# nikola3794/normal-clustering-nerf

Measured on AMD Instinct MI355X. Metric: training rays/sec (+ samples/sec), higher is better.
Workload: dtype fp32 (march/composite/losses); fp16-operand MFMA with fp32 accumulate in the field MLP; 1 GPU; configs[1]+[2]: full training step, 8192 rays/GPU, normal clustering on; rays_per_gpu=8192, global_batch=8192, grid=128, max_samples=1024, parallelism=dp1, grid_update_every_16=True

## Files before the change

normal-clustering-nerf_amd/csrc/optim.hip:

```cpp
#include <algorithm>
#include "workgroup.h"
#include "../../include/ncnerf.h"

namespace ncn {

constexpr int SUMSQ_BLOCKS = 1024;

__global__ __launch_bounds__(256) void sumsq_kernel(const float* __restrict__ x, int64_t n, float* __restrict__ part,
                                                    int* __restrict__ step_inc) {
    __shared__ float red[4];
    if (step_inc && blockIdx.x == 0 && threadIdx.x == 0) *step_inc += 1;
    float s = 0.f;
    const int64_t n4 = n / 4;
    const float4* x4 = (const float4*)x;
    for (int64_t i = (int64_t)blockIdx.x * 256 + threadIdx.x; i < n4; i += (int64_t)gridDim.x * 256) {
        const float4 v = x4[i];
        s = fmaf(v.x, v.x, s); s = fmaf(v.y, v.y, s); s = fmaf(v.z, v.z, s); s = fmaf(v.w, v.w, s);
    }
    if (blockIdx.x == 0)
        for (int64_t i = n4 * 4 + threadIdx.x; i < n; i += 256) s = fmaf(x[i], x[i], s);
    s = block_sum<256>(s, red);
    if (threadIdx.x == 0) part[blockIdx.x] = s;
}

__device__ __forceinline__ float clip_coef(const float* __restrict__ part, float max_norm) {
    __shared__ float c_s;
    if (threadIdx.x < 64) {
        float s = 0.f;
        for (int i = threadIdx.x; i < SUMSQ_BLOCKS; i += 64) s += part[i];
        s = wave_sum(s);
        if (threadIdx.x == 0) {
            const float norm = sqrtf(s);
            const float c = max_norm / (norm + 1e-6f);
            c_s = max_norm > 0.f ? fminf(c, 1.0f) : 1.0f;
        }
    }
    __syncthreads();
    return c_s;
}

__global__ __launch_bounds__(256) void adam_kernel(float* __restrict__ p, const float* __restrict__ g,
                                                   float* __restrict__ m, float* __restrict__ v, int64_t n,
                                                   const float* __restrict__ part, float max_norm, float lr, float b1,
                                                   float b2, float eps, float wd, float bc1, float bc2,
                                                   const float* __restrict__ lr_dev, const int* __restrict__ step_dev) {
    const float cf = part ? clip_coef(part, max_norm) : 1.0f;
    if (lr_dev) lr = *lr_dev;
    if (step_dev) {
        const float st = (float)*step_dev;
        bc1 = 1.0f - powf(b1, st);
        bc2 = 1.0f - powf(b2, st);
    }
    auto upd = [&](float& pi, float gr, float& mi, float& vi) {
        const float gi = gr * cf;
        mi = b1 * mi + (1.f - b1) * gi;
        vi = b2 * vi + (1.f - b2) * gi * gi;
        const float denom = sqrtf(vi / bc2) + eps;
        pi = pi - lr * ((mi / bc1) / denom + wd * pi);
    };
    const int64_t tid = (int64_t)blockIdx.x * 256 + threadIdx.x, nth = (int64_t)gridDim.x * 256;
    const bool vec = (((uintptr_t)p | (uintptr_t)g | (uintptr_t)m | (uintptr_t)v) & 15) == 0;
    const int64_t n4 = vec ? n / 4 : 0;
    for (int64_t i = tid; i < n4; i += nth) {
        float4 P = ((float4*)p)[i], M = ((float4*)m)[i], V = ((float4*)v)[i];
        const float4 G = ((const float4*)g)[i];
        upd(P.x, G.x, M.x, V.x);
        upd(P.y, G.y, M.y, V.y);
        upd(P.z, G.z, M.z, V.z);
        upd(P.w, G.w, M.w, V.w);
        ((float4*)p)[i] = P;
        ((float4*)m)[i] = M;
        ((float4*)v)[i] = V;
    }
    for (int64_t i = 4 * n4 + tid; i < n; i += nth) upd(p[i], g[i], m[i], v[i]);
}

#ifndef NCN_ADAM_BLOCKS
#define NCN_ADAM_BLOCKS 256
#endif
#ifndef NCN_ADAM_UNROLL
#define NCN_ADAM_UNROLL 12
#endif
constexpr int ADAM_BLOCKS = NCN_ADAM_BLOCKS;
constexpr int ADAM_THREADS = 1024;
constexpr int ADAM_UNROLL = NCN_ADAM_UNROLL;
__global__ __launch_bounds__(ADAM_THREADS) void adam_prep_kernel(const float* __restrict__ g, int64_t n, float gscale,
                                                               float max_norm, double b1, double b2, float lr,
                                                               const float* __restrict__ lr_dev,
                                                               int* __restrict__ step_dev, float* __restrict__ work,
                                                               float* __restrict__ amp, const int* __restrict__ gate) {
    float* part = work;
    unsigned* cnt = (unsigned*)(work + ADAM_BLOCKS);
    float* sc = work + ADAM_BLOCKS + 4;
    __shared__ float red[ADAM_THREADS / 64];
    const int64_t n4 = n / 4, stride = (int64_t)gridDim.x * ADAM_THREADS;
    const float4* g4 = (const float4*)g;
    float s = 0.f;
    for (int64_t b = (int64_t)blockIdx.x * ADAM_THREADS + threadIdx.x; b < n4; b += ADAM_UNROLL * stride) {
        float4 x[ADAM_UNROLL];
#pragma unroll
        for (int u = 0; u < ADAM_UNROLL; u++) x[u] = b + u * stride < n4 ? g4[b + u * stride] : make_float4(0, 0, 0, 0);
#pragma unroll
        for (int u = 0; u < ADAM_UNROLL; u++) {
            s = fmaf(x[u].x, x[u].x, s); s = fmaf(x[u].y, x[u].y, s); s = fmaf(x[u].z, x[u].z, s); s = fmaf(x[u].w, x[u].w, s);
        }
    }
    if (blockIdx.x == 0)
        for (int64_t i = 4 * n4 + threadIdx.x; i < n; i += ADAM_THREADS) s = fmaf(g[i], g[i], s);
    if (!last_block_arrive(&part[blockIdx.x], block_sum<ADAM_THREADS>(s, red), cnt)) return;
    if (threadIdx.x < 64) {
        float q[ADAM_BLOCKS / 64];
#pragma unroll
        for (int u = 0; u < ADAM_BLOCKS / 64; u++) {
            const int i = u * 64 + threadIdx.x;
            q[u] = i < (int)gridDim.x ? __hip_atomic_load(&part[i], __ATOMIC_RELAXED, __HIP_MEMORY_SCOPE_AGENT) : 0.f;
        }
        float t = 0.f;
#pragma unroll
        for (int u = 0; u < ADAM_BLOCKS / 64; u++) t += q[u];
        t = wave_sum(t);
        if (threadIdx.x == 0) {
            const float c = max_norm / (sqrtf(t) * gscale + 1e-6f);
            const bool gated_off = gate && *gate == 0;
            const bool skip = gated_off || (amp && !isfinite(t));
            if (amp && !gated_off) {
                float tr = skip ? 0.f : amp[1] + 1.f;
                float scale = skip ? amp[0] * 0.5f : amp[0];
                if (tr >= (float)NCN_AMP_GROWTH_INTERVAL) {
                    scale *= 2.f;
                    tr = 0.f;
                }
                amp[0] = scale;
                amp[1] = tr;
            }
            const int st = *step_dev + (skip ? 0 : 1);
            *step_dev = st;
            sc[4] = skip ? 1.f : 0.f;
            sc[0] = (max_norm > 0.f ? fminf(c, 1.0f) : 1.0f) * gscale;
            sc[1] = (float)(1.0 - pow(b1, (double)st));
            sc[2] = (float)(1.0 - pow(b2, (double)st));
            sc[3] = lr_dev ? *lr_dev : lr;
            *cnt = 0u;
        }
    }
}
template <int PK>
__device__ __forceinline__ void adam_pack1(int64_t e, float x, const int32_t* __restrict__ pinv, int64_t poff,
                                           int64_t n, void* __restrict__ packed) {
    if (PK == 0 || e < poff || e >= n) return;
    const int64_t w = e - poff;
    const int2 q = ((const int2*)pinv)[w];
    if (PK == 1) {
        const _Float16 h = (_Float16)x;
        if (q.x >= 0) ((_Float16*)packed)[q.x] = h;
        if (q.y >= 0) ((_Float16*)packed)[q.y] = h;
    } else {
        const __bf16 h = (__bf16)x;
        if (q.x >= 0) ((__bf16*)packed)[q.x] = h;
        if (q.y >= 0) ((__bf16*)packed)[q.y] = h;
    }
}
template <bool ZERO, int PK>
__global__ __launch_bounds__(256) void adam_apply_kernel(float* __restrict__ p, float* __restrict__ g,
                                                         float* __restrict__ m, float* __restrict__ v, int64_t n,
                                                         int64_t n0, float b1, float b2, float eps, float wd0,
                                                         float wd1, const float* __restrict__ sc,
                                                         const int32_t* __restrict__ pinv, int64_t poff,
                                                         void* __restrict__ packed) {
    const float cf = sc[0], bc1 = sc[1], bc2 = sc[2], lr = sc[3];
    if (sc[4] != 0.f) {
        if (PK) {
            const int64_t tid = (int64_t)blockIdx.x * 256 + threadIdx.x, nth = (int64_t)gridDim.x * 256;
            for (int64_t e = poff + tid; e < n; e += nth) adam_pack1<PK>(e, p[e], pinv, poff, n, packed);
        }
        if (ZERO) {
            const int64_t tid = (int64_t)blockIdx.x * 256 + threadIdx.x, nth = (int64_t)gridDim.x * 256;
            for (int64_t i = tid; i < n / 4; i += nth) ((float4*)g)[i] = make_float4(0.f, 0.f, 0.f, 0.f);
            for (int64_t i = 4 * (n / 4) + tid; i < n; i += nth) g[i] = 0.f;
        }
        return;
    }
    auto upd = [&](float& pi, float gr, float& mi, float& vi, float wd) {
        const float gi = gr * cf;
        mi = b1 * mi + (1.f - b1) * gi;
        vi = b2 * vi + (1.f - b2) * gi * gi;
        const float denom = sqrtf(vi / bc2) + eps;
        pi = pi - lr * ((mi / bc1) / denom + wd * pi);
    };
    auto upd_tail = [&](float& pi, float gr, float& mi, float& vi, float wd) {
#pragma clang fp contract(off)
        const float gi = gr * cf;
        mi = fmaf(b1, mi, (1.f - b1) * gi);
        vi = fmaf(b2, vi, ((1.f - b2) * gi) * gi);
        const float denom = sqrtf(vi / bc2) + eps;
        pi = fmaf(-lr, fmaf(wd, pi, (mi / bc1) / denom), pi);
    };
    const int64_t n4 = n / 4, tid = (int64_t)blockIdx.x * 256 + threadIdx.x, nth = (int64_t)gridDim.x * 256;
#pragma unroll 2
    for (int64_t i = tid; i < n4; i += nth) {
        float4 P = ((float4*)p)[i], M = ((float4*)m)[i], V = ((float4*)v)[i];
        const float4 G = ((const float4*)g)[i];
        const int64_t e = 4 * i;
        upd(P.x, G.x, M.x, V.x, e < n0 ? wd0 : wd1);
        upd(P.y, G.y, M.y, V.y, e + 1 < n0 ? wd0 : wd1);
        upd(P.z, G.z, M.z, V.z, e + 2 < n0 ? wd0 : wd1);
        upd(P.w, G.w, M.w, V.w, e + 3 < n0 ? wd0 : wd1);
        ((float4*)p)[i] = P;
        ((float4*)m)[i] = M;
        ((float4*)v)[i] = V;
        if (PK && e + 3 >= poff) {
            adam_pack1<PK>(e, P.x, pinv, poff, n, packed);
            adam_pack1<PK>(e + 1, P.y, pinv, poff, n, packed);
            adam_pack1<PK>(e + 2, P.z, pinv, poff, n, packed);
            adam_pack1<PK>(e + 3, P.w, pinv, poff, n, packed);
        }
        if (ZERO && (G.x != 0.f || G.y != 0.f || G.z != 0.f || G.w != 0.f))
            ((float4*)g)[i] = make_float4(0.f, 0.f, 0.f, 0.f);
    }
    for (int64_t i = 4 * n4 + tid; i < n; i += nth) {
        upd_tail(p[i], g[i], m[i], v[i], i < n0 ? wd0 : wd1);
        adam_pack1<PK>(i, p[i], pinv, poff, n, packed);
        if (ZERO) g[i] = 0.f;
    }
}
constexpr int NCN_STEP_MAX_BUFS = 8;
struct StepCopies {
    const unsigned char* src[NCN_STEP_MAX_BUFS];
    unsigned char* dst[NCN_STEP_MAX_BUFS];
    int64_t bytes[NCN_STEP_MAX_BUFS];
};
__global__ __launch_bounds__(256) void step_inputs_kernel(StepCopies c, int nb, int64_t* step_dst, int64_t step,
                                                         int* flag_dst, int flag) {
    if (step_dst && blockIdx.x == 0 && threadIdx.x == 0) *step_dst = step;
    if (flag_dst && blockIdx.x == 0 && threadIdx.x == 0) *flag_dst = flag;
    const int64_t tid = (int64_t)blockIdx.x * 256 + threadIdx.x, nth = (int64_t)gridDim.x * 256;
    for (int b = 0; b < nb; b++) {
        const bool al = (((uintptr_t)c.src[b] | (uintptr_t)c.dst[b]) & 15) == 0;
        const int64_t n16 = al ? c.bytes[b] / 16 : 0;
        for (int64_t i = tid; i < n16; i += nth) ((uint4*)c.dst[b])[i] = ((const uint4*)c.src[b])[i];
        for (int64_t i = 16 * n16 + tid; i < c.bytes[b]; i += nth) c.dst[b][i] = c.src[b][i];
    }
}

__global__ __launch_bounds__(256) void grad_pack_f16_kernel(const float* __restrict__ g, int64_t n,
                                                            const float* __restrict__ scale, int world,
                                                            _Float16* __restrict__ w) {
    const float s = scale ? *scale : 1.f, wf = (float)world;
    auto wire = [&](float x) { return (_Float16)((float)(_Float16)(x * s) / wf); };
    const int64_t n8 = n / 8, stride = (int64_t)gridDim.x * 256;
    for (int64_t i = (int64_t)blockIdx.x * 256 + threadIdx.x; i < n8; i += stride) {
        const float4 a = ((const float4*)g)[2 * i], b = ((const float4*)g)[2 * i + 1];
        typedef _Float16 h8 __attribute__((ext_vector_type(8)));
        const h8 o = {wire(a.x), wire(a.y), wire(a.z), wire(a.w), wire(b.x), wire(b.y), wire(b.z), wire(b.w)};
        ((h8*)w)[i] = o;
    }
    for (int64_t i = 8 * n8 + (int64_t)blockIdx.x * 256 + threadIdx.x; i < n; i += stride) w[i] = wire(g[i]);
}
__global__ __launch_bounds__(256) void grad_unpack_f16_kernel(const _Float16* __restrict__ w, int64_t n,
                                                              const float* __restrict__ scale, float* __restrict__ g) {
    const float inv = scale ? 1.f / *scale : 1.f;
    const int64_t n8 = n / 8, stride = (int64_t)gridDim.x * 256;
    typedef _Float16 h8 __attribute__((ext_vector_type(8)));
    for (int64_t i = (int64_t)blockIdx.x * 256 + threadIdx.x; i < n8; i += stride) {
        const h8 v = ((const h8*)w)[i];
        ((float4*)g)[2 * i] = make_float4((float)v[0] * inv, (float)v[1] * inv, (float)v[2] * inv, (float)v[3] * inv);
        ((float4*)g)[2 * i + 1] = make_float4((float)v[4] * inv, (float)v[5] * inv, (float)v[6] * inv, (float)v[7] * inv);
    }
    for (int64_t i = 8 * n8 + (int64_t)blockIdx.x * 256 + threadIdx.x; i < n; i += stride) g[i] = (float)w[i] * inv;
}

}

using namespace ncn;

extern "C" {

int ncn_grad_pack_f16(const float* grad, int64_t n, const float* scale, int world, uint16_t* wire, void* stream) {
    if (n <= 0) return 0;
    NCN_REQUIRE(world >= 1, hipErrorInvalidValue, "ncn_grad_pack_f16: world must be >= 1");
    NCN_REQUIRE(((((uintptr_t)grad) & 15) | (((uintptr_t)wire) & 15)) == 0, hipErrorInvalidValue,
                "ncn_grad_pack_f16: grad and wire must be 16-byte aligned");
    const int blocks = (int)std::min<int64_t>(std::max<int64_t>(1, cdiv(n, 2048)), 4096);
    hipLaunchKernelGGL(grad_pack_f16_kernel, dim3(blocks), dim3(256), 0, (hipStream_t)stream, grad, n, scale,
                       world, (_Float16*)wire);
    NCN_LAUNCH_CHECK("ncn_grad_pack_f16");
    return 0;
}

int ncn_grad_unpack_f16(const uint16_t* wire, int64_t n, const float* scale, float* grad, void* stream) {
    if (n <= 0) return 0;
    NCN_REQUIRE(((((uintptr_t)grad) & 15) | (((uintptr_t)wire) & 15)) == 0, hipErrorInvalidValue,
                "ncn_grad_unpack_f16: grad and wire must be 16-byte aligned");
    const int blocks = (int)std::min<int64_t>(std::max<int64_t>(1, cdiv(n, 2048)), 4096);
    hipLaunchKernelGGL(grad_unpack_f16_kernel, dim3(blocks), dim3(256), 0, (hipStream_t)stream, (const _Float16*)wire,
                       n, scale, grad);
    NCN_LAUNCH_CHECK("ncn_grad_unpack_f16");
    return 0;
}

int ncn_step_inputs(int n_bufs, const void* const* src, void* const* dst, const int64_t* n_bytes, int64_t* step_dst,
                    int64_t step, int32_t* flag_dst, int32_t flag, void* stream) {
    NCN_REQUIRE(n_bufs >= 0 && n_bufs <= NCN_STEP_MAX_BUFS, hipErrorInvalidValue,
                "ncn_step_inputs: at most 8 buffers");
    StepCopies c{};
    int64_t total = 0;
    for (int b = 0; b < n_bufs; b++) {
        NCN_REQUIRE(n_bytes[b] >= 0 && (n_bytes[b] == 0 || (src[b] && dst[b])), hipErrorInvalidValue,
                    "ncn_step_inputs: null buffer");
        c.src[b] = (const unsigned char*)src[b];
        c.dst[b] = (unsigned char*)dst[b];
        c.bytes[b] = n_bytes[b];
        total += n_bytes[b];
    }
    const int grid = (int)std::max<int64_t>(1, std::min<int64_t>(256, (total / 16 + 255) / 256));
    hipLaunchKernelGGL(step_inputs_kernel, dim3(grid), dim3(256), 0, (hipStream_t)stream, c, n_bufs, step_dst, step,
                       flag_dst, flag);
    NCN_LAUNCH_CHECK("ncn_step_inputs");
    return 0;
}

int ncn_sumsq(const float* x, int64_t n, float* out_partial, int* step_inc, void* stream) {
    hipLaunchKernelGGL(sumsq_kernel, dim3(SUMSQ_BLOCKS), dim3(256), 0, (hipStream_t)stream, x, n, out_partial,
                       step_inc);
    NCN_LAUNCH_CHECK("ncn_sumsq");
    return 0;
}

int ncn_adam(float* params, const float* grads, float* exp_avg, float* exp_avg_sq, int64_t n,
             const float* sumsq_partial, float max_norm, float lr, float beta1, float beta2, float eps,
             float weight_decay, int step, const float* lr_dev, const int* step_dev, void* stream) {
    if (n <= 0) return 0;
    NCN_REQUIRE(step >= 1 || step_dev, hipErrorInvalidValue, "ncn_adam: step must be >= 1");
    const float bc1 = 1.0f - powf(beta1, (float)std::max(step, 1)), bc2 = 1.0f - powf(beta2, (float)std::max(step, 1));
    const int blocks = (int)std::min<int64_t>(cdiv(n, 1024), 2048);
    hipLaunchKernelGGL(adam_kernel, dim3(blocks), dim3(256), 0, (hipStream_t)stream, params, grads, exp_avg,
                       exp_avg_sq, n, sumsq_partial, max_norm, lr, beta1, beta2, eps, weight_decay, bc1, bc2, lr_dev,
                       step_dev);
    NCN_LAUNCH_CHECK("ncn_adam");
    return 0;
}

}

template <int PK>
static void launch_apply(int zero, int blocks, hipStream_t st, float* params, float* grads, float* exp_avg,
                         float* exp_avg_sq, int64_t n, int64_t n_group0, double beta1, double beta2, float eps,
                         float wd0, float wd1, const float* sc, const int32_t* pinv, int64_t poff, void* packed) {
    if (zero)
        hipLaunchKernelGGL((adam_apply_kernel<true, PK>), dim3(blocks), dim3(256), 0, st, params, grads, exp_avg,
                           exp_avg_sq, n, n_group0, (float)beta1, (float)beta2, eps, wd0, wd1, sc, pinv, poff, packed);
    else
        hipLaunchKernelGGL((adam_apply_kernel<false, PK>), dim3(blocks), dim3(256), 0, st, params, grads, exp_avg,
                           exp_avg_sq, n, n_group0, (float)beta1, (float)beta2, eps, wd0, wd1, sc, pinv, poff, packed);
}

static int adam_step_impl(float* params, float* grads, float* exp_avg, float* exp_avg_sq, int64_t n, int64_t n_group0,
                          float grad_scale, float max_norm, float lr, double beta1, double beta2, float eps, float wd0,
                          float wd1, const float* lr_dev, int* step_dev, float* work, int zero_grads,
                          float* amp_state, const int* gate, const int32_t* pinv, int64_t poff, void* packed, int pk,
                          void* stream) {
    if (n <= 0) return 0;
    NCN_REQUIRE(((((uintptr_t)params) | ((uintptr_t)grads) | ((uintptr_t)exp_avg) | ((uintptr_t)exp_avg_sq)) & 15) == 0,
                hipErrorInvalidValue, "ncn_adam_step: buffers must be 16-byte aligned");
    NCN_REQUIRE(step_dev != nullptr && work != nullptr, hipErrorInvalidValue,
                "ncn_adam_step: needs the device step counter and the work buffer");
    const int prep_blocks = (int)std::min<int64_t>(ADAM_BLOCKS, std::max<int64_t>(1, cdiv(n / 4, ADAM_THREADS * 4)));
    hipLaunchKernelGGL(adam_prep_kernel, dim3(prep_blocks), dim3(ADAM_THREADS), 0, (hipStream_t)stream, grads, n,
                       grad_scale, max_norm, beta1, beta2, lr, lr_dev, step_dev, work, amp_state, gate);
    NCN_LAUNCH_CHECK("ncn_adam_step (prep)");
    const int blocks = (int)std::min<int64_t>(std::max<int64_t>(1, cdiv(n, 2048)), 16384);
    const float* sc = work + ADAM_BLOCKS + 4;
    const hipStream_t st = (hipStream_t)stream;
    if (pk == 0)
        launch_apply<0>(zero_grads, blocks, st, params, grads, exp_avg, exp_avg_sq, n, n_group0, beta1, beta2, eps, wd0,
                        wd1, sc, nullptr, 0, nullptr);
    else if (pk == 1)
        launch_apply<1>(zero_grads, blocks, st, params, grads, exp_avg, exp_avg_sq, n, n_group0, beta1, beta2, eps, wd0,
                        wd1, sc, pinv, poff, packed);
    else
        launch_apply<2>(zero_grads, blocks, st, params, grads, exp_avg, exp_avg_sq, n, n_group0, beta1, beta2, eps, wd0,
                        wd1, sc, pinv, poff, packed);
    NCN_LAUNCH_CHECK("ncn_adam_step");
    return 0;
}

extern "C" {

int ncn_adam_step(float* params, float* grads, float* exp_avg, float* exp_avg_sq, int64_t n, int64_t n_group0,
                  float grad_scale, float max_norm, float lr, double beta1, double beta2, float eps, float wd0, float wd1,
                  const float* lr_dev, int* step_dev, float* work, int zero_grads, float* amp_state, const int* gate,
                  void* stream) {
    return adam_step_impl(params, grads, exp_avg, exp_avg_sq, n, n_group0, grad_scale, max_norm, lr, beta1, beta2, eps,
                          wd0, wd1, lr_dev, step_dev, work, zero_grads, amp_state, gate, nullptr, 0, nullptr, 0, stream);
}

int ncn_adam_step_packed(float* params, float* grads, float* exp_avg, float* exp_avg_sq, int64_t n, int64_t n_group0,
                         float grad_scale, float max_norm, float lr, double beta1, double beta2, float eps, float wd0,
                         float wd1, const float* lr_dev, int* step_dev, float* work, int zero_grads, float* amp_state,
                         const int* gate, const int32_t* pack_inv, int64_t pack_off, uint16_t* packed, int pack_prec,
                         void* stream) {
    NCN_REQUIRE(pack_inv && packed && (pack_prec == NCN_PREC_F16 || pack_prec == NCN_PREC_BF16) && pack_off >= 0 &&
                    n - pack_off == NCN_FIELD_NW && (((uintptr_t)pack_inv) & 7) == 0,
                hipErrorInvalidValue, "ncn_adam_step_packed: pack_inv/packed/pack_prec/pack_off invalid");
    return adam_step_impl(params, grads, exp_avg, exp_avg_sq, n, n_group0, grad_scale, max_norm, lr, beta1, beta2, eps,
                          wd0, wd1, lr_dev, step_dev, work, zero_grads, amp_state, gate, pack_inv, pack_off, packed,
                          pack_prec == NCN_PREC_F16 ? 1 : 2, stream);
}

int64_t ncn_adam_step_work_floats(void) { return ADAM_BLOCKS + 12; }

}
```

normal-clustering-nerf_amd/csrc/vren_march_pack.h:

```cpp
#pragma once
#include "vren_march_wave.h"
#include "workgroup.h"

namespace ncn {

__global__ __launch_bounds__(1024) void march_train_scan_kernel(const int32_t* __restrict__ counts, int64_t R,
                                                                int64_t* __restrict__ rays_a,
                                                                int32_t* __restrict__ counter) {
    __shared__ int wave_tot[16];
    const int tid = threadIdx.x;
    int carry = 0;
    for (int64_t base = 0; base < R; base += 4096) {
        const int64_t i0 = base + (int64_t)tid * 4;
        int c[4];
        int local = 0;
#pragma unroll
        for (int j = 0; j < 4; j++) {
            c[j] = (i0 + j < R) ? counts[i0 + j] : 0;
            local += c[j];
        }
        int run = block_excl_sweep<1024>(local, carry, wave_tot);
#pragma unroll
        for (int j = 0; j < 4; j++) {
            const int64_t i = i0 + j;
            if (i < R) {
                rays_a[3 * i] = i;
                rays_a[3 * i + 1] = run;
                rays_a[3 * i + 2] = c[j];
            }
            run += c[j];
        }
    }
    if (tid == 0) {
        counter[0] = carry;
        counter[1] = (int32_t)R;
    }
}

__device__ __forceinline__ void copy_slab_row(const float* __restrict__ sx, const float* __restrict__ st,
                                              const float* __restrict__ sd, const float (&d3)[3], int k0, int n,
                                              int64_t start, int lane, float* __restrict__ xyzs,
                                              float* __restrict__ dirs, float* __restrict__ deltas,
                                              float* __restrict__ ts) {
    for (int k = 3 * k0 + lane; k < 3 * n; k += 64) {
        xyzs[3 * start + k] = sx[k];
        dirs[3 * start + k] = d3[k % 3];
    }
    for (int k = k0 + lane; k < n; k += 64) {
        ts[start + k] = st[k];
        deltas[start + k] = sd[k];
    }
}

__global__ __launch_bounds__(256) void march_train_pack_kernel(
    const float* __restrict__ rays_d, const int64_t* __restrict__ rays_a, int64_t R, int max_samples,
    const float* __restrict__ slab_xyz, const float* __restrict__ slab_t, const float* __restrict__ slab_dt,
    float* __restrict__ xyzs, float* __restrict__ dirs, float* __restrict__ deltas, float* __restrict__ ts) {
    const int lane = threadIdx.x & 63;
    const int64_t n = __builtin_amdgcn_readfirstlane((int)(blockIdx.x * 4 + (threadIdx.x >> 6)));
    if (n >= R) return;
    const int64_t ray = rays_a[3 * n], start = rays_a[3 * n + 1];
    const int cnt = (int)rays_a[3 * n + 2];
    const float d3[3] = {rays_d[3 * ray], rays_d[3 * ray + 1], rays_d[3 * ray + 2]};
    copy_slab_row(slab_xyz + ray * (int64_t)max_samples * 3, slab_t + ray * (int64_t)max_samples,
                  slab_dt + ray * (int64_t)max_samples, d3, 0, cnt, start, lane, xyzs, dirs, deltas, ts);
}

__global__ __launch_bounds__(256) void march_train_place_kernel(
    const float* __restrict__ rays_d, int64_t R, int max_samples, const int32_t* __restrict__ counts,
    const int32_t* __restrict__ wg_sum, const float* __restrict__ slab_xyz, const float* __restrict__ slab_t,
    const float* __restrict__ slab_dt, int64_t* __restrict__ rays_a, float* __restrict__ xyzs,
    float* __restrict__ dirs, float* __restrict__ deltas, float* __restrict__ ts, int32_t* __restrict__ counter) {
    __shared__ int red[4][3];
    const int lane = threadIdx.x & 63, wv = threadIdx.x >> 6;
    const int b = blockIdx.x;
    int v[PLACE_MAX_WG / 256];
#pragma unroll
    for (int u = 0; u < PLACE_MAX_WG / 256; u++) {
        const int i = u * 256 + threadIdx.x;
        v[u] = i < (int)gridDim.x ? wg_sum[i] : 0;
    }
    const int64_t r0 = __builtin_amdgcn_readfirstlane((int)(b * 4 + wv));
    const bool live = r0 < R;
    const int64_t r = live ? r0 : R - 1;
    const int n = live ? counts[r] : 0;
    const float d3[3] = {rays_d[3 * r], rays_d[3 * r + 1], rays_d[3 * r + 2]};
    const float* sx = slab_xyz + r * (int64_t)max_samples * 3;
    const float* st = slab_t + r * (int64_t)max_samples;
    const float* sd = slab_dt + r * (int64_t)max_samples;
    constexpr int PF = 4;
    float px[3 * PF], pt[PF], pd[PF];
#pragma unroll
    for (int q = 0; q < 3 * PF; q++) px[q] = q * 64 + lane < 3 * n ? sx[q * 64 + lane] : 0.f;
#pragma unroll
    for (int q = 0; q < PF; q++) {
        pt[q] = q * 64 + lane < n ? st[q * 64 + lane] : 0.f;
        pd[q] = q * 64 + lane < n ? sd[q * 64 + lane] : 0.f;
    }
    int pre[3] = {0, 0, 0};
#pragma unroll
    for (int u = 0; u < PLACE_MAX_WG / 256; u++) {
        const int i = u * 256 + threadIdx.x;
        const int nl = (int)((unsigned)v[u] >> 26);
        if (i < b) {
            pre[0] += v[u] & ((1 << 26) - 1);
            pre[1] += nl;
        }
        pre[2] += nl;
    }
    block_sum<3, 256>(pre, red);
    int start = pre[0];
    const int long_before = pre[1], long_total = pre[2];
    __syncthreads();
    int* const len = &red[0][0];
    if (lane == 0) len[wv] = n;
    __syncthreads();
    int lw = 0;
    for (int w = 0; w < wv; w++) {
        start += len[w];
        lw += len[w] > PLACE_LONG;
    }
    const int64_t row = n > PLACE_LONG ? (int64_t)(long_before + lw)
                                       : (int64_t)long_total + (4 * (int64_t)b - long_before) + (wv - lw);
    if (b == (int)gridDim.x - 1 && threadIdx.x == 0) {
        counter[0] = start + len[0] + len[1] + len[2] + len[3];
        counter[1] = (int32_t)R;
    }
    if (!live) return;
    if (lane == 0) {
        rays_a[3 * row] = r;
        rays_a[3 * row + 1] = start;
        rays_a[3 * row + 2] = n;
    }
    float* ox = xyzs + 3 * (int64_t)start;
    float* od = dirs + 3 * (int64_t)start;
#pragma unroll
    for (int q = 0; q < 3 * PF; q++) {
        const int k = q * 64 + lane;
        if (k < 3 * n) {
            ox[k] = px[q];
            od[k] = d3[k % 3];
        }
    }
#pragma unroll
    for (int q = 0; q < PF; q++) {
        const int k = q * 64 + lane;
        if (k < n) {
            ts[start + k] = pt[q];
            deltas[start + k] = pd[q];
        }
    }
    copy_slab_row(sx, st, sd, d3, PF * 64, n, start, lane, xyzs, dirs, deltas, ts);
}

}
```

normal-clustering-nerf_amd/csrc/vren_march_wave.h:

```cpp
#pragma once
#include "vren_aabb.h"
#include "vren_march.h"

namespace ncn {


template <int P>
__device__ __forceinline__ float march_chain(float cb, float dt, int lane, float (&c)[P]) {
    constexpr int L = 64 * P;
#pragma unroll
    for (int j = 0; j < P; j++) c[j] = cb;
    int j0 = 0;
    float v = cb;
    for (;;) {
        const uint32_t bv = __float_as_uint(v);
        const float v1 = v + dt;
        const uint32_t b1 = __float_as_uint(v1);
        uint32_t r1 = b1 - bv, r = 0;
        int K;
        float vn;
        if ((bv >> 23) != (b1 >> 23) || bv == 0u) {
            K = 0;
            vn = v1;
        } else {
            const float v2 = v1 + dt;
            const uint32_t b2 = __float_as_uint(v2);
            if ((b2 >> 23) != (b1 >> 23)) {
                K = 1;
                vn = v2;
            } else {
                r = b2 - b1;
                if (r == 0u) {
#pragma unroll
                    for (int j = 0; j < P; j++)
                        if (lane + 64 * j > j0) c[j] = v;
                    return v;
                }
                const uint32_t room = (bv | 0x7FFFFFu) - bv - r1;
                K = (uint64_t)room >= (uint64_t)(L - 1) * r ? L : (int)(room / r + 1u);
                vn = __uint_as_float(bv + r1 + (uint32_t)(K - 1) * r) + dt;
            }
        }
#pragma unroll
        for (int j = 0; j < P; j++) {
            const int i = lane + 64 * j;
            if (i > j0 && i <= j0 + K) c[j] = __uint_as_float(bv + r1 + (uint32_t)(i - j0 - 1) * r);
        }
        if (j0 + K >= L) return __uint_as_float(bv + r1 + (uint32_t)(L - j0 - 1) * r);
        const int J = j0 + K + 1;
        if (J == L) return vn;
#pragma unroll
        for (int j = 0; j < P; j++)
            if (lane + 64 * j == J) c[j] = vn;
        j0 = J;
        v = vn;
    }
}

__device__ __forceinline__ float lane_f(float v, int idx) { return __int_as_float(__builtin_amdgcn_ds_bpermute(idx << 2, __float_as_int(v))); }
__device__ __forceinline__ int lane_i(int v, int idx) { return __builtin_amdgcn_ds_bpermute(idx << 2, v); }

__device__ __forceinline__ int march_skip_lane(float c, float T, float dt, int lane) {
    const float q = ceilf((T - c) / dt);
    int j = lane + (int)fminf(fmaxf(q, 1.0f), 65.0f);
    if (j > 64) j = 64;
    const float cm = lane_f(c, min(j - 1, 63));
    const float cj = lane_f(c, min(j, 63));
    if (j - 1 > lane && cm >= T) j -= 1;
    else if (j < 64 && cj < T) j += 1;
    const float cm2 = lane_f(c, min(j - 1, 63));
    const float cj2 = lane_f(c, min(j, 63));
    const bool ok = (j - 1 == lane || cm2 < T) && (j == 64 || cj2 >= T);
    if (__ballot(!ok)) {
        int p = lane;
#pragma unroll
        for (int st = 32; st >= 1; st >>= 1) {
            const int qn = p + st;
            const float cq = lane_f(c, min(qn, 63));
            if (qn <= 63 && cq < T) p = qn;
        }
        j = p + 1;
    }
    return j;
}

__device__ __forceinline__ uint64_t march_visited(int nxt, int s, int lane) {
    int J[6];
    J[0] = nxt;
#pragma unroll
    for (int i = 1; i < 6; i++) {
        const int v = lane_i(J[i - 1], min(J[i - 1], 63));
        J[i] = J[i - 1] >= 64 ? 64 : v;
    }
    int cur = s;
#pragma unroll
    for (int i = 5; i >= 0; i--) {
        const int v = lane_i(J[i], min(cur, 63));
        const int cand = cur >= 64 ? 64 : v;
        if (cand <= lane) cur = cand;
    }
    return __ballot(cur == lane && lane >= s);
}

template <bool ONE_CASCADE, int P>
__device__ __forceinline__ int march_walk_wave(const MarchConst& m, const uint8_t* __restrict__ bitfield, float ox,
                                               float oy, float oz, float dx, float dy, float dz, float t1, float t2,
                                               float noise_r, float dt, int lane, float* __restrict__ sx,
                                               float* __restrict__ st, float* __restrict__ sd) {
    const float dxi = 1.0f / dx, dyi = 1.0f / dy, dzi = 1.0f / dz;
    int n = 0;
    if (t1 >= 0) {
        t1 = fmaf(dt, noise_r, t1);
        float cb = t1;
        bool pend = false, done = false;
        float ptgt = 0.f;
        int s = 0;
        for (int it = 0; it < (1 << 16) && !done; it++) {
            float c[P];
            const float cnext = march_chain<P>(cb, dt, lane, c);
            float X[P], Y[P], Z[P], tgt[P];
            bool occ[P];
#pragma unroll
            for (int j = 0; j < P; j++) {
                X[j] = fmaf(c[j], dx, ox);
                Y[j] = fmaf(c[j], dy, oy);
                Z[j] = fmaf(c[j], dz, oz);
                int nx, ny, nz;
                float mip_bound;
                uint32_t cbi = 0xFFFFFFFFu, cbv = 0;
                occ[j] = probe<ONE_CASCADE>(m, bitfield, X[j], Y[j], Z[j], dt, nx, ny, nz, mip_bound, cbi, cbv);
                tgt[j] = skip_target(m, c[j], X[j], Y[j], Z[j], dx, dy, dz, dxi, dyi, dzi, nx, ny, nz, mip_bound);
            }
#pragma unroll
            for (int j = 0; j < P; j++) {
                if (done) break;
                const uint64_t lt_m = __ballot(c[j] < t2);
                const uint64_t occ_m = __ballot(occ[j]);
                if (pend) {
                    const uint64_t mm = __ballot(c[j] >= ptgt);
                    if (!mm) continue;
                    s = __builtin_ctzll(mm);
                    pend = false;
                }
                const int skip = march_skip_lane(c[j], tgt[j], dt, lane);
                const int nxt = !(c[j] < t2) ? 64 : (occ[j] ? lane + 1 : skip);
                const uint64_t vis = march_visited(nxt, s, lane);
                const uint64_t term = vis & ~lt_m;
                uint64_t emit = vis & occ_m & lt_m;
                const int room = m.max_samples - n;
                if (__popcll(emit) >= room) {
                    uint64_t e2 = emit;
                    for (int q = 1; q < room; q++) e2 &= e2 - 1;
                    const int last = __builtin_ctzll(e2);
                    emit &= (last == 63) ? ~0ull : ((2ull << last) - 1);
                    done = true;
                }
                if (term) {
                    emit &= (1ull << __builtin_ctzll(term)) - 1;
                    done = true;
                }
                if (emit) {
                    if ((emit >> lane) & 1) {
                        const int k = n + (int)__builtin_amdgcn_mbcnt_hi((uint32_t)(emit >> 32),
                                                                       __builtin_amdgcn_mbcnt_lo((uint32_t)emit, 0));
                        sx[3 * k] = X[j];
                        sx[3 * k + 1] = Y[j];
                        sx[3 * k + 2] = Z[j];
                        st[k] = c[j];
                        sd[k] = dt;
                    }
                    n += __popcll(emit);
                }
                if (!done) {
                    const int lastv = 63 - __builtin_clzll(vis);
                    if ((occ_m >> lastv) & 1) {
                        s = 0;
                    } else {
                        pend = true;
                        ptgt = __int_as_float(__builtin_amdgcn_readlane(__float_as_int(tgt[j]), lastv));
                    }
                }
            }
            cb = cnext;
        }
    }
    return n;
}

template <bool ONE_CASCADE, int P>
__global__ __launch_bounds__(256) void march_train_wave_kernel(
    const float* __restrict__ rays_o, const float* __restrict__ rays_d, const float* __restrict__ hits_t,
    const float* __restrict__ noise, int64_t R, const uint8_t* __restrict__ bitfield, int cascades, float scale,
    int G, int max_samples, int32_t* __restrict__ counts, float* __restrict__ slab_xyz,
    float* __restrict__ slab_t, float* __restrict__ slab_dt) {
    const int lane = threadIdx.x & 63;
    const int64_t r = __builtin_amdgcn_readfirstlane((int)(blockIdx.x * 4 + (threadIdx.x >> 6)));
    if (r >= R) return;
    const MarchConst m = make_march_const(cascades, scale, 0.0f, G, max_samples, scale);
    const float t1 = hits_t[2 * r];
    const int n = march_walk_wave<ONE_CASCADE, P>(
        m, bitfield, rays_o[3 * r], rays_o[3 * r + 1], rays_o[3 * r + 2], rays_d[3 * r], rays_d[3 * r + 1],
        rays_d[3 * r + 2], t1, hits_t[2 * r + 1], t1 >= 0 ? noise[r] : 0.f, calc_dt(m, 0.0f), lane,
        slab_xyz + r * (int64_t)max_samples * 3, slab_t + r * (int64_t)max_samples, slab_dt + r * (int64_t)max_samples);
    if (lane == 0) counts[r] = n;
}

__device__ __forceinline__ float march_uniform(uint64_t seed, uint64_t ctr, uint32_t r) {
    uint64_t z = seed + 0x9E3779B97F4A7C15ull * (ctr * 0x100000001B3ull + r + 1u);
    z = (z ^ (z >> 30)) * 0xBF58476D1CE4E5B9ull;
    z = (z ^ (z >> 27)) * 0x94D049BB133111EBull;
    z ^= z >> 31;
    return (float)(uint32_t)(z >> 40) * (1.0f / 16777216.0f);
}

constexpr int PLACE_MAX_WG = 256 * 16;
constexpr int PLACE_LONG = 256;

template <bool ONE_CASCADE, int P>
__global__ __launch_bounds__(256) void march_train_walk2_kernel(
    const float* __restrict__ rays_o, const float* __restrict__ rays_d, int64_t R, float cx, float cy, float cz,
    float hx, float hy, float hz, float near_distance, const float* __restrict__ noise, uint64_t seed,
    const int64_t* __restrict__ rng_ctr, const uint8_t* __restrict__ bitfield, int cascades, float scale, int G,
    int max_samples, float* __restrict__ slab_xyz, float* __restrict__ slab_t, float* __restrict__ slab_dt,
    int32_t* __restrict__ counts, int32_t* __restrict__ wg_sum) {
    __shared__ int cnt_s[4];
    const int lane = threadIdx.x & 63, wv = threadIdx.x >> 6;
    const int64_t r0 = __builtin_amdgcn_readfirstlane((int)(blockIdx.x * 4 + wv));
    const bool live = r0 < R;
    const int64_t r = live ? r0 : R - 1;
    const MarchConst m = make_march_const(cascades, scale, 0.0f, G, max_samples, scale);
    const float o[3] = {rays_o[3 * r], rays_o[3 * r + 1], rays_o[3 * r + 2]};
    const float d[3] = {rays_d[3 * r], rays_d[3 * r + 1], rays_d[3 * r + 2]};
    const float c3[3] = {cx, cy, cz}, h3[3] = {hx, hy, hz};
    const float inv[3] = {1.0f / d[0], 1.0f / d[1], 1.0f / d[2]};
    float t1, t2;
    slab_test(o, inv, c3, h3, t1, t2);
    if (t2 > 0) t1 = fmaxf(t1, 0.0f);
    else { t1 = -1.0f; t2 = -1.0f; }
    if (t1 >= 0.0f && t1 < near_distance) t1 = near_distance;
    float nz = 0.f;
    if (t1 >= 0) nz = noise ? noise[r] : march_uniform(seed, rng_ctr ? (uint64_t)*rng_ctr : 0ull, (uint32_t)r);
    int n = 0;
    if (live)
        n = march_walk_wave<ONE_CASCADE, P>(m, bitfield, o[0], o[1], o[2], d[0], d[1], d[2], t1, t2, nz,
                                            calc_dt(m, 0.0f), lane, slab_xyz + r * (int64_t)max_samples * 3,
                                            slab_t + r * (int64_t)max_samples, slab_dt + r * (int64_t)max_samples);
    if (lane == 0) {
        cnt_s[wv] = n;
        if (live) counts[r] = n;
    }
    __syncthreads();
    if (threadIdx.x == 0) {
        int nl = 0;
#pragma unroll
        for (int w = 0; w < 4; w++) nl += cnt_s[w] > PLACE_LONG;
        wg_sum[blockIdx.x] = (cnt_s[0] + cnt_s[1] + cnt_s[2] + cnt_s[3]) | (nl << 26);
    }
}

}
```

normal-clustering-nerf_amd/ncnerf_amd/_lib.py:

```python
import ctypes
import operator
import os
import re

import torch

_HERE = os.path.dirname(os.path.abspath(__file__))
LIB_PATH = os.environ.get("NCN_LIB_PATH") or os.path.join(_HERE, "libncnerf.so")
INCLUDE_DIR = os.path.join(os.path.dirname(os.path.dirname(_HERE)), "include")
_DERIVED = {
    "ncnerf.h": "the binding",
    "ncnerf_metrics.h": "the binding of the validation metrics",
    "ncnerf_geom.h": "the binding of the geometry supervision",
    "ncnerf_mesh.h": "the binding of the isosurface extraction",
    "ncnerf_heads.h": "the binding of the semantic / normal heads",
    "ncnerf_sem.h": "the binding of the semantic metrics",
    "ncnerf_input_grad.h": "the binding of the split backward's direction gradient",
}
HEADERS = tuple(_DERIVED)

P = ctypes.c_void_p
I64 = ctypes.c_int64
I32 = ctypes.c_int
U32 = ctypes.c_uint32
F32 = ctypes.c_float
F64 = ctypes.c_double
U64 = ctypes.c_uint64


class NcnError(RuntimeError):
    pass


_RESTYPES = {"int": ctypes.c_int, "int64_t": I64, "const char*": ctypes.c_char_p}
_SCALARS = {"int": I32, "int32_t": I32, "int64_t": I64, "uint32_t": U32, "uint64_t": U64, "float": F32, "double": F64}
_POINTEES = {"void": 0, "float": 4, "double": 8, "int": 4, "int32_t": 4, "int64_t": 8, "uint8_t": 1, "uint16_t": 2,
             "uint32_t": 4}
_DECL = re.compile(r"(const\s+char\s*\*|int64_t|int)\s*(\w+)\s*\(([^()]*)\)")
_PARAM = re.compile(r"(?:const\s+)?(\w+)(?:\s*((?:\*\s*(?:const\b\s*)?)+)|\s+)(\w+)")


def parse_header(text):
    text = re.sub(r"/\*.*?\*/|//[^\n]*", " ", text, flags=re.S)
    if re.search(r"^\s*#.*\\$", text, flags=re.M):
        raise ValueError("ncnerf.h grammar: a preprocessor line is continued with a backslash")
    text = re.sub(r"^\s*#.*$", "", text, flags=re.M)
    text, n_extern = re.subn(r'extern\s+"C"\s*\{', "", text)
    text = text.strip()
    if n_extern == 1 and text.endswith("}"):
        text = text[:-1]
    *decls, rest = text.split(";")
    if rest.strip():
        raise ValueError(f"ncnerf.h grammar: no ';' after {' '.join(rest.split())!r}")
    out = {}
    for decl in decls:
        decl = " ".join(decl.split())
        m = _DECL.fullmatch(decl)
        if m is None:
            raise ValueError(f"ncnerf.h grammar: not `int|int64_t|const char* name(params)`: {decl!r}")
        ret, name, params = m.groups()
        if name in out:
            raise ValueError(f"ncnerf.h grammar: {name} is declared twice")
        plist = []
        for p in ([] if params.strip() in ("", "void") else params.split(",")):
            pm = _PARAM.fullmatch(p.strip())
            if pm is None or pm.group(3) in _POINTEES or pm.group(3) in _SCALARS or pm.group(3) == "const":
                raise ValueError(f"ncnerf.h grammar: parameter {p.strip()!r} of {decl!r} is not `type name`")
            base, stars, pname = pm.group(1), (pm.group(2) or "").count("*"), pm.group(3)
            if stars == 0 and base in _SCALARS:
                plist.append((base, 0, pname))
            elif stars == 1 and base in _POINTEES:
                plist.append(("ptr", _POINTEES[base], pname))
            elif stars == 2 and base == "void":
                plist.append(("ptr", 8, pname))
            else:
                raise ValueError(f"ncnerf.h grammar: unknown type in parameter {p.strip()!r} of {decl!r}")
        out[name] = ("const char*" if ret.startswith("const") else ret, plist)
    return out


def header_path(name, include_dir=INCLUDE_DIR):
    return os.path.join(include_dir, name)


def read_header(name, include_dir=INCLUDE_DIR):
    path = header_path(name, include_dir)
    try:
        return open(path).read()
    except OSError as e:
        raise NcnError(f"include/{name} not found at {path}: {_DERIVED[name]} is derived from it ({e})") from None


_DEFINE = re.compile(r"^[ \t]*#[ \t]*define[ \t]+(NCN_\w+)(.*)$", flags=re.M)
_INT = re.compile(r"[+-]?(?:0|[1-9]\d*)")
_FLOAT = re.compile(r"[+-]?(?:(?:\d+\.\d*|\.\d+)(?:[eE][+-]?\d+)?|\d+[eE][+-]?\d+)[fF]?")


def parse_constants(text):
    text = re.sub(r"/\*.*?\*/|//[^\n]*", " ", text, flags=re.S)
    constants, left_out = {}, []
    for name, body in _DEFINE.findall(text):
        body = body.strip()
        if name in constants or name in left_out:
            raise ValueError(f"ncnerf.h grammar: {name} is defined twice")
        if _INT.fullmatch(body):
            constants[name] = int(body)
        elif _FLOAT.fullmatch(body):
            constants[name] = float(body.rstrip("fF"))
        else:
            left_out.append(name)
    return constants, left_out


def load_headers(include_dir=INCLUDE_DIR):
    abi, header_of, constants, left_out = {}, {}, {}, []
    for header in HEADERS:
        text = read_header(header, include_dir)
        decls = parse_header(text)
        values, opaque = parse_constants(text)
        for name in (*decls, *values, *opaque):
            if name in header_of:
                raise NcnError(f"{name} is declared in include/{header} and in include/{header_of[name]}")
            header_of[name] = header
        abi.update(decls)
        constants.update(values)
        left_out += opaque
    return abi, header_of, constants, tuple(left_out)


ABI, HEADER_OF, CONSTANTS, NON_LITERAL_DEFINES = load_headers()
AMP_INIT_SCALE = CONSTANTS["NCN_AMP_INIT_SCALE"]


def declaration(name):
    return ABI[name]


def symbols(header=None):
    if header is not None and header not in HEADERS:
        raise KeyError(header)
    return [name for name in ABI if header is None or HEADER_OF[name] == header]


def exported_symbols():
    return symbols()


SIGNATURES = {name: [P if kind == "ptr" else _SCALARS[kind] for kind, _, _ in params]
              for name, (_, params) in ABI.items()}

_lib = None

TIMING = None
TIMING_SPIN_CYCLES = 60000


def lib():
    global _lib
    if _lib is None:
        if not os.path.exists(LIB_PATH):
            raise NcnError(f"libncnerf.so not found at {LIB_PATH}: run __graft_entry__.build() "
                           f"(make -C normal-clustering-nerf_amd)")
        L = ctypes.CDLL(LIB_PATH)
        for name, (ret, _) in ABI.items():
            fn = getattr(L, name)
            fn.argtypes = SIGNATURES[name]
            fn.restype = _RESTYPES[ret]
        _lib = L
    return _lib


_Tensor = torch.Tensor
_CTYPES = (ctypes.c_int.__mro__[-2], type(ctypes.byref(ctypes.c_int())))
_AUTO = object()


def _launches(params):
    return bool(params) and params[-1] == ("ptr", 0, "stream")


def _refuse(name, i, a):
    params = declaration(name)[1]
    kind, width, pname = params[i]
    expected = f"a host {kind}" if kind != "ptr" else (
        f"a {'CUDA ' if _launches(params) else ''}tensor{' of %d-byte elements' % width if width else ''}, "
        f"None or a ctypes pointer")
    got = f"a {a.dtype} {a.device.type} tensor" if isinstance(a, _Tensor) else f"{type(a).__name__} {a!r}"
    raise TypeError(f"{name}: argument {i} ({pname}) takes {expected}, got {got}")


def _number(name, i, a, convert):
    if isinstance(a, (_Tensor, str, bytes, bytearray)):
        _refuse(name, i, a)
    try:
        return convert(a)
    except TypeError:
        _refuse(name, i, a)


def _marshal_source(name, params):
    launches = _launches(params)
    n = len(params)
    src = [f"def marshal({', '.join(f'a{i}' for i in range(n))}{'=_AUTO' if launches else ''}):"]
    for i, (kind, width, _) in enumerate(params):
        a = f"a{i}"
        if kind == "ptr":
            bad = ([f"{a}.element_size() != {width}"] if width else []) + ([f"not {a}.is_cuda"] if launches else [])
            auto = launches and i == n - 1
            src += [f" if {a} is _AUTO: {a} = stream()"] if auto else []
            src += [f" {'el' if auto else ''}if isinstance({a}, _Tensor):"]
            src += [f"  if {' or '.join(bad)}: _refuse({name!r}, {i}, {a})"] if bad else []
            src += [f"  {a} = {a}.data_ptr()",
                    f" elif {a} is not None and not isinstance({a}, _CTYPES): _refuse({name!r}, {i}, {a})"]
        else:
            exact, convert = ("float", "float") if kind in ("float", "double") else ("int", "operator.index")
            src += [f" if type({a}) is not {exact} and not isinstance({a}, _CTYPES):"
                    f" {a} = _number({name!r}, {i}, {a}, {convert})"]
    src += [f" return ({''.join(f'a{i}, ' for i in range(n))})"]
    return "\n".join(src)


def _marshaller(name, params):
    ns = {}
    exec(_marshal_source(name, params), globals(), ns)
    n = len(params)
    return ns["marshal"], (n - 1, n) if _launches(params) else (n,)


_PLANS = {name: _marshaller(name, params) for name, (_, params) in ABI.items()}


def marshal(name, args):
    fn, counts = _PLANS[name]
    if len(args) not in counts:
        decl = ", ".join(f"{'pointer' if kind == 'ptr' else kind} {pname}" for kind, _, pname in declaration(name)[1])
        raise TypeError(f"{name}: takes {' or '.join(map(str, counts))} arguments, got {len(args)}: {name}({decl})")
    return fn(*args)


def call(name, *args):
    args = marshal(name, args)
    if TIMING is not None and name in TIMING:
        e0 = torch.cuda.Event(enable_timing=True)
        e1 = torch.cuda.Event(enable_timing=True)
        torch.cuda._sleep(TIMING_SPIN_CYCLES)
        e0.record()
        rc = getattr(lib(), name)(*args)
        e1.record()
        TIMING[name].append((e0, e1))
    else:
        rc = getattr(lib(), name)(*args)
    if rc != 0:
        msg = lib().ncn_last_error().decode(errors="replace")
        raise NcnError(f"{name} failed (hipError {rc}): {msg}")
    return rc


def stream():
    return P(torch.cuda.current_stream().cuda_stream)


def ptr(t):
    if t is None:
        return P(None)
    return P(t.data_ptr())


def step_inputs(srcs, dsts, step_dev, step, flag_dev=None, flag=0):
    n = len(srcs)
    VP = ctypes.c_void_p * max(n, 1)
    src = VP(*[s.data_ptr() for s in srcs])
    dst = VP(*[d.data_ptr() for d in dsts])
    nb = (ctypes.c_int64 * max(n, 1))(*[s.numel() * s.element_size() for s in srcs])
    return call("ncn_step_inputs", n, src, dst, nb, step_dev, int(step), flag_dev, int(flag))


def check_input(t, name):
    if not isinstance(t, torch.Tensor) or not t.is_cuda:
        raise RuntimeError(f"{name} must be a CUDA tensor")
    if not t.is_contiguous():
        raise RuntimeError(f"{name} must be contiguous")


def check_dtype(t, dtype, name):
    if t.dtype != dtype:
        raise RuntimeError(f"{name} must be {dtype} (got {t.dtype})")
```

normal-clustering-nerf_amd/ncnerf_amd/ngp_mt.py:

```python
import math

import numpy as np
import torch
from einops import rearrange
from torch import nn

from . import _lib, vren
from ._lib import CONSTANTS as _C, call

L_LEVELS, F_PER_LEVEL, LOG2_T, N_MIN = 16, 2, 19, 16
MLP_SHAPES = ((64, 32), (16, 64), (64, 32), (64, 64), (16, 64))
N_W = sum(o * i for o, i in MLP_SHAPES)
PRECISIONS = {"fp16": _C["NCN_PREC_F16"], "bf16": _C["NCN_PREC_BF16"]}
N_PACKED_HALVES = _C["NCN_FIELD_PACKED_HALVES"]
ENC_BYTES = _C["NCN_ENC_BYTES_PER_SAMPLE"]
SORT_MIN_SAMPLES = 8192
W_SIGMA = 64 * 32 + 16 * 64
W_RGB = N_W - W_SIGMA
HEAD_MAX_OUT = _C["NCN_HEAD_MAX_OUT"]
N_HEAD_PACKED_HALVES = _C["NCN_HEAD_PACKED_HALVES"]


def head_shapes(n_out):
    if not isinstance(n_out, int) or isinstance(n_out, bool) or not 1 <= n_out <= HEAD_MAX_OUT:
        raise ValueError(f"a head has 1..{HEAD_MAX_OUT} outputs (got {n_out!r})")
    return ((64, 16), (64, 64), (16 * ((n_out + 15) // 16), 64))


def head_nw(n_out):
    return sum(o * i for o, i in head_shapes(n_out))


def grid_levels(scale, n_levels=L_LEVELS, log2_T=LOG2_T, n_min=N_MIN):
    b = math.exp(math.log(2048 * scale / n_min) / (n_levels - 1))
    log2_pls = np.float32(np.log2(np.float32(b)))
    levels, offset = [], 0
    for l in range(n_levels):
        s = np.float32(np.float32(np.exp2(np.float32(l) * log2_pls)) * np.float32(n_min) - np.float32(1.0))
        res = int(math.ceil(float(s))) + 1
        params = min(((res ** 3 + 7) // 8) * 8, 1 << log2_T)
        levels.append(dict(scale=float(s), res=res, params=params, offset=offset))
        offset += params
    return levels, offset


def level_words(levels):
    w = np.zeros(64, np.uint32)
    for l, lv in enumerate(levels):
        w[4 * l] = np.frombuffer(np.float32(lv["scale"]).tobytes(), np.uint32)[0]
        w[4 * l + 1], w[4 * l + 2], w[4 * l + 3] = lv["res"], lv["params"], lv["offset"]
    return w


class _ParamHolder(nn.Module):

    def __init__(self, flat_view):
        super().__init__()
        self.params = nn.Parameter(flat_view)


class _FieldFunction(torch.autograd.Function):

    @staticmethod
    def forward(ctx, x, d, table, w_sigma, w_rgb, model, mode, n_dev=None):
        need_grad = any(ctx.needs_input_grad[:5])
        sigmas, rgbs, enc, packed, order = model._field_fwd(x, d, n_dev, mode, need_grad)
        if need_grad:
            need_in = ctx.needs_input_grad[0] or (d is not None and ctx.needs_input_grad[1])
            ctx.save_for_backward(x, d, enc, packed, n_dev, order, table if need_in else None)
            ctx.model = model
        if mode != 0:
            ctx.mark_non_differentiable(rgbs)
        ctx.set_materialize_grads(False)
        return sigmas, rgbs

    @staticmethod
    def backward(ctx, dL_dsigmas, dL_drgbs):
        x, d, enc, packed, n_dev, order, table = ctx.saved_tensors
        model = ctx.model
        n = x.shape[0]
        dev = x.device
        need_x = ctx.needs_input_grad[0]
        need_d = d is not None and ctx.needs_input_grad[1]
        need_param = any(ctx.needs_input_grad[2:5])
        L = _lib.lib()
        dE_ws = torch.empty(int(L.ncn_field_bwd_dE_floats(n)), dtype=torch.float32, device=dev)
        c = lambda t: None if t is None else t.contiguous().float()
        dsig, drgb = c(dL_dsigmas), c(dL_drgbs)
        scale = model._bwd_loss_scale()
        g_table, g_w = model._grad_views() if need_param else (None, None)
        dL_dx = dL_dd = None
        if d is None:
            nb = int(L.ncn_field_bwd_part_blocks(n, 2))
            slab = torch.empty(nb * N_W, dtype=torch.float32, device=dev)
            stash = torch.zeros(int(L.ncn_field_bwd_stash_floats(n)), dtype=torch.float32, device=dev)
            lmax = model._level_max()
            lmax.zero_()
            dE_ws[:4].zero_()
            call("ncn_field_bwd_mlp_part", x, None, n, n_dev, order, packed, model._prec, enc, dsig, None, None, scale,
                 2, 0, slab, dE_ws, lmax, stash)
            if need_param:
                model._scatter(x, n, n_dev, order, dE_ws, lmax, g_table)
                call("ncn_field_reduce_wgrad_parts", slab, nb, 0, g_w)
        else:
            nb = L.ncn_field_bwd_blocks(n)
            slab = torch.empty(nb * N_W, dtype=torch.float32, device=dev)
            lmax = model._level_max()
            if need_param and not (need_x or need_d) and model.scatter_split is None:
                call("ncn_field_bwd", x, d, n, n_dev, order, model._levels_ptr, model._xyz_min, model._xyz_extent,
                     packed, model._prec, enc, dsig, drgb, scale, g_table, slab, dE_ws, lmax)
            else:
                if need_d:
                    dL_dd = torch.empty(n, 3, dtype=torch.float32, device=dev)
                    call("ncn_field_bwd_mlp_din", x, d, n, n_dev, order, packed, model._prec, enc, dsig, drgb, scale,
                         slab, dE_ws, lmax, model._flat[model._n_table:], dL_dd)
                else:
                    call("ncn_field_bwd_mlp", x, d, n, n_dev, order, packed, model._prec,
                         enc, dsig, drgb, scale, slab, dE_ws, lmax)
                if need_param:
                    model._scatter(x, n, n_dev, order, dE_ws, lmax, g_table)
            if need_param:
                call("ncn_field_reduce_wgrad", slab, nb, g_w)
        if need_x:
            dL_dx = torch.empty(n, 3, dtype=torch.float32, device=dev)
            call("ncn_field_bwd_dx", x, n, n_dev, order, table, model._levels_ptr,
                 model._xyz_min, model._xyz_extent, dE_ws, dL_dx)
        return dL_dx, dL_dd, None, None, None, None, None, None


class _FieldHeadsFunction(torch.autograd.Function):

    @staticmethod
    def forward(ctx, x, d, n_dev, model, *params):
        need_in = ctx.needs_input_grad[0] or ctx.needs_input_grad[1]
        need_grad = need_in or any(ctx.needs_input_grad[4:])
        sigmas, rgbs, enc, packed, _ = model._field_fwd(x, d, n_dev, 0, True)
        n = x.shape[0]
        outs = []
        for name, n_out, _, _ in model._heads:
            o = torch.empty(n, n_out, dtype=torch.float32, device=x.device)
            if n > 0:
                call("ncn_head_fwd", enc, n, n_dev, packed, model._head_packed[name], n_out, model._prec, o)
            outs.append(o)
        if need_grad:
            ctx.save_for_backward(x, d, enc, packed, n_dev, model.xyz_encoder.params if need_in else None,
                                  *[model._head_packed[h[0]] for h in model._heads])
            ctx.model = model
        ctx.set_materialize_grads(False)
        return (sigmas, rgbs) + tuple(outs)

    @staticmethod
    def backward(ctx, dL_dsigmas, dL_drgbs, *dL_dheads):
        x, d, enc, packed, n_dev, table, *head_packed = ctx.saved_tensors
        model = ctx.model
        n, dev = x.shape[0], x.device
        need_x, need_d = ctx.needs_input_grad[0], ctx.needs_input_grad[1]
        need_param = any(ctx.needs_input_grad[4:])
        none = (None,) * (2 + 3 + len(model._heads))
        if n == 0:
            return (torch.zeros_like(x) if need_x else None, torch.zeros_like(d) if need_d else None) + none
        L = _lib.lib()
        c = lambda t: None if t is None else t.contiguous().float()
        scale = model._bwd_loss_scale()
        g_table, g_w = model._grad_views() if need_param else (None, None)
        nb = (int(L.ncn_field_bwd_part_blocks(n, 1)), int(L.ncn_field_bwd_part_blocks(n, 2)))
        slab = torch.empty(max(nb) * N_W, dtype=torch.float32, device=dev)
        dE_ws = torch.empty(int(L.ncn_field_bwd_dE_floats(n)), dtype=torch.float32, device=dev)
        stash = torch.empty(int(L.ncn_field_bwd_stash_floats(n)), dtype=torch.float32, device=dev)
        lmax = model._level_max()
        dL_dx = dL_dd = None
        if need_d:
            dL_dd = torch.empty(n, 3, dtype=torch.float32, device=dev)
            call("ncn_field_bwd_mlp_rgb_din", x, d, n, n_dev, None, packed, model._prec, enc, c(dL_drgbs), scale, nb[0],
                 slab, dE_ws, lmax, stash, model._flat[model._n_table:], dL_dd)
        else:
            call("ncn_field_bwd_mlp_part", x, d, n, n_dev, None, packed, model._prec, enc, None, None, c(dL_drgbs),
                 scale, 1, nb[0], slab, dE_ws, lmax, stash)
        nbh = int(L.ncn_head_bwd_blocks(n))
        for (name, n_out, off, n_w), hp, g in zip(model._heads, head_packed, dL_dheads):
            if g is None:
                continue
            hslab = torch.empty(nbh * n_w, dtype=torch.float32, device=dev)
            call("ncn_head_bwd", enc, n, n_dev, packed, hp, n_out, model._prec, c(g), scale, hslab, stash)
            if need_param:
                call("ncn_head_reduce_wgrad", hslab, nbh, n_w, model._flat_grad[off:off + n_w])
        call("ncn_field_bwd_mlp_part", x, d, n, n_dev, None, packed, model._prec, enc, c(dL_dsigmas), None, None, scale,
             2, nb[1], slab, dE_ws, lmax, stash)
        if need_param:
            model._scatter(x, n, n_dev, None, dE_ws, lmax, g_table, wgrad=(slab, nb[1], nb[0], g_w))
        if need_x:
            dL_dx = torch.empty(n, 3, dtype=torch.float32, device=dev)
            call("ncn_field_bwd_dx", x, n, n_dev, None, table, model._levels_ptr, model._xyz_min, model._xyz_extent,
                 dE_ws, dL_dx)
        return (dL_dx, dL_dd) + none


class NGPMT(nn.Module):
    def _bwd_loss_scale(self):
        return self.amp_state if self.amp_state is not None else self._amp_unit

    def _level_max(self):
        dev = self._flat.device
        if self.scatter_split is not None:
            return torch.empty(16 * 256, dtype=torch.float32, device=dev)
        if getattr(self, "_lmax", None) is None or self._lmax.device != dev:
            self._lmax = torch.empty(16 * 256, dtype=torch.float32, device=dev)
        return self._lmax

    def __init__(self, scale, grid_size, rgb_act="Sigmoid", pred_sem=False, pred_norm=False, seed=1337,
                 precision="fp16", amp="internal", **kwargs):
        super().__init__()
        if precision not in PRECISIONS:
            raise ValueError(f"precision must be one of {sorted(PRECISIONS)}")
        if amp not in ("internal", "external"):
            raise ValueError("amp must be 'internal' or 'external'")
        self.amp = amp
        self.precision = precision
        self._prec = PRECISIONS[precision]
        if rgb_act != "Sigmoid":
            raise NotImplementedError("rgb_act='None' (exposure tonemappers) is off in every reference config")
        pred_sem, pred_norm = bool(pred_sem), bool(pred_norm)
        heads = []
        if pred_sem:
            if kwargs.get("n_sem_cls") is None:
                raise NotImplementedError("pred_sem=True needs the class count: pass n_sem_cls (the reference reads "
                                          "kwargs['n_sem_cls'], ngp_mt.py:119)")
            head_shapes(kwargs["n_sem_cls"])
            heads.append(("sem_net", kwargs["n_sem_cls"]))
            self.n_sem_cls = kwargs["n_sem_cls"]
        if pred_norm:
            heads.append(("norm_net", 3))
        self.pred_sem, self.pred_norm, self.rgb_act = pred_sem, pred_norm, rgb_act
        self.scale = scale
        self.register_buffer("center", torch.zeros(1, 3))
        self.register_buffer("xyz_min", -torch.ones(1, 3) * scale)
        self.register_buffer("xyz_max", torch.ones(1, 3) * scale)
        self.register_buffer("half_size", (self.xyz_max - self.xyz_min) / 2)
        self._aabb = (tuple(float(v) for v in self.center[0]), tuple(float(v) for v in self.half_size[0]))
        self.cascades = max(1 + int(np.ceil(np.log2(2 * scale))), 1)
        self.grid_size = grid_size
        self.register_buffer("density_bitfield", torch.zeros(self.cascades * grid_size ** 3 // 8, dtype=torch.uint8))
        self.levels, self.n_entries = grid_levels(scale)
        self._level_words = level_words(self.levels)
        self._levels_ptr = self._level_words.ctypes.data_as(_lib.P)
        self._xyz_min = float(np.float32(-scale))
        self._xyz_extent = float(np.float32(scale) - np.float32(-scale))
        n_table = self.n_entries * F_PER_LEVEL
        self._n_table = n_table
        self._heads, off = [], n_table + N_W
        for name, n_out in heads:
            self._heads.append((name, n_out, off, head_nw(n_out)))
            off += head_nw(n_out)
        flat = torch.zeros(off)
        g = torch.Generator().manual_seed(seed)
        flat[:n_table] = (torch.rand(n_table, generator=g) * 2 - 1) * 1e-4
        off = n_table
        for o, i in MLP_SHAPES:
            a = math.sqrt(6.0 / (o + i))
            flat[off:off + o * i] = (torch.rand(o * i, generator=g) * 2 - 1) * a
            off += o * i
        for _, n_out, _, _ in self._heads:
            for o, i in head_shapes(n_out):
                a = math.sqrt(6.0 / (o + i))
                flat[off:off + o * i] = (torch.rand(o * i, generator=g) * 2 - 1) * a
                off += o * i
        self._flat = flat
        self.xyz_encoder = _ParamHolder(flat[:n_table])
        self.sigma_net = _ParamHolder(flat[n_table:n_table + W_SIGMA])
        self.rgb_net = _ParamHolder(flat[n_table + W_SIGMA:n_table + N_W])
        for name, _, off, n_w in self._heads:
            setattr(self, name, _ParamHolder(flat[off:off + n_w]))
        self._flat_grad = None
        self._packed = None
        self._head_packed = {}
        f16 = precision == "fp16"
        self.register_buffer("amp_state", torch.tensor([_lib.AMP_INIT_SCALE, 0.0]) if f16 and amp == "internal" else None)
        self.register_buffer("_amp_unit", torch.ones(1) if f16 and amp == "external" else None, persistent=False)
        self.scatter_split = None
        self.sort_samples = False
        self._deferred = []
        self._deferred_graph = []

    def _param_slices(self):
        n_table = self._n_table
        return ([(self.xyz_encoder.params, 0, n_table), (self.sigma_net.params, n_table, n_table + W_SIGMA),
                 (self.rgb_net.params, n_table + W_SIGMA, n_table + N_W)]
                + [(getattr(self, name).params, off, off + n_w) for name, _, off, n_w in self._heads])

    def _apply(self, fn, recurse=True):
        super()._apply(fn, recurse)
        flat = fn(self._flat)
        for p, a, b in self._param_slices():
            flat[a:b].copy_(p.data)
        self._flat = flat
        for p, a, b in self._param_slices():
            p.data = flat[a:b]
        self._flat_grad = None
        self._packed = None
        self._head_packed = {}
        return self

    def flat_params(self):
        return self._flat

    def flat_grad(self):
        self._grad_views()
        return self._flat_grad

    def _grad_views(self):
        if self._flat_grad is None or self._flat_grad.device != self._flat.device:
            self._flat_grad = torch.zeros_like(self._flat)
        fg, n_table = self._flat_grad, self._n_table
        for p, a, b in self._param_slices():
            v = fg[a:b]
            if p.grad is None or p.grad.data_ptr() != v.data_ptr():
                if p.grad is not None:
                    v.copy_(p.grad)
                else:
                    v.zero_()
                p.grad = v
        return fg[:n_table], fg[n_table:n_table + N_W]

    def grad_buckets(self, split):
        fg = self.flat_grad()
        cut = 2 * self.levels[split]["offset"]
        return fg[cut:], fg[:cut]

    def run_deferred_scatter(self, max_blocks=0, graph=False):
        entries = self._deferred_graph if graph else self._deferred
        if not entries:
            raise RuntimeError("run_deferred_scatter: no deferred scatter (scatter_split unset or no backward yet)")
        for x, n, n_dev, order, dE_ws, lmax, g_table in entries:
            call("ncn_field_scatter", x, n, n_dev, order, self._levels_ptr, self._xyz_min, self._xyz_extent, dE_ws,
                 lmax, 0, self.scatter_split, max_blocks, g_table)
        if not graph:
            self._deferred = []

    def prepare_weights(self):
        self._pack_weights()
        self._packed_fresh = True

    def _load_from_state_dict(self, *args, **kwargs):
        super()._load_from_state_dict(*args, **kwargs)
        self._packed_fresh = False

    def _take_packed(self):
        if getattr(self, "_packed_fresh", False) and self._packed is not None:
            self._packed_fresh = False
            return self._packed
        return self._pack_weights()

    def pack_target(self):
        if self._heads:
            raise RuntimeError("pack_target: ncn_adam_step_packed refreshes the field's fragments only; a model with "
                               "heads takes ncn_adam_step and packs explicitly (FlatAdam does)")
        if self._packed is None or self._packed.device != self._flat.device:
            self._pack_weights()
        inv = getattr(self, "_pack_inv", None)
        if inv is None or inv.device != self._flat.device:
            src = torch.empty(N_PACKED_HALVES, dtype=torch.int32, device=self._flat.device)
            call("ncn_field_pack_map", src)
            s = src.cpu().numpy()
            table = np.full((N_W, 2), -1, np.int32)
            fill = np.zeros(N_W, np.int64)
            for q, w in enumerate(s):
                assert 0 <= w < N_W and fill[w] < 2, (q, w)
                table[w, fill[w]] = q
                fill[w] += 1
            inv = self._pack_inv = torch.from_numpy(table).to(self._flat.device)
        return inv, self._n_table, self._packed, self._prec

    def _pack_weights(self):
        if self._packed is None or self._packed.device != self._flat.device:
            self._packed = torch.empty(N_PACKED_HALVES, dtype=torch.float16, device=self._flat.device)
        call("ncn_field_pack_weights", self._flat[self._n_table:], self._packed, self._prec)
        for name, n_out, off, n_w in self._heads:
            hp = self._head_packed.get(name)
            if hp is None or hp.device != self._flat.device:
                hp = self._head_packed[name] = torch.empty(N_HEAD_PACKED_HALVES, dtype=torch.float16,
                                                           device=self._flat.device)
            call("ncn_head_pack_weights", self._flat[off:off + n_w], n_out, hp, self._prec)
        return self._packed

    def _field_fwd(self, x, d, n_dev, mode, need_grad):
        n = x.shape[0]
        dev = x.device
        sigmas = torch.empty(n, dtype=torch.float32, device=dev)
        rgbs = torch.empty(n, 3, dtype=torch.float32, device=dev) if mode == 0 else sigmas.new_empty(0, 3)
        enc = None
        if need_grad:
            enc = torch.empty(((n + 15) // 16) * 16 * ENC_BYTES // 2, dtype=torch.float16, device=dev)
        packed = self._take_packed()
        order = None
        if self._heads and self.sort_samples:
            raise NotImplementedError("sort_samples (the Morton-window processing order) is not supported with a "
                                      "pred_sem / pred_norm head")
        if need_grad and self.sort_samples and n >= SORT_MIN_SAMPLES:
            order = torch.empty(n, dtype=torch.int32, device=dev)
            call("ncn_field_sort_windows", x, n, n_dev, self._xyz_min, self._xyz_extent, order)
        call("ncn_field_fwd", x, d if mode == 0 else None, n, n_dev, order, self.xyz_encoder.params, self._levels_ptr,
             self._xyz_min, self._xyz_extent, packed, self._prec, mode, sigmas, rgbs if mode == 0 else None, enc)
        return sigmas, rgbs, enc, packed, order

    def _scatter(self, x, n, n_dev, order, dE_ws, lmax, g_table, wgrad=None):
        split = self.scatter_split
        lo = 0 if split is None else split
        slab, nb_s, nb_r, g_w = wgrad if wgrad is not None else (None, 0, 0, None)
        call("ncn_field_scatter_wgrad", x, n, n_dev, order, self._levels_ptr, self._xyz_min, self._xyz_extent, dE_ws,
             lmax, lo, 16, 0, g_table, slab, nb_s, nb_r, g_w)
        if split is not None:
            self._deferred.append((x, n, n_dev, order, dE_ws, lmax, g_table))

    def density(self, x, return_feat=False):
        _lib.check_input(x, "x")
        if return_feat:
            return self._density_feat(x.float().contiguous())
        sigmas, _ = _FieldFunction.apply(x.float().contiguous(), None, self.xyz_encoder.params,
                                         self.sigma_net.params, self.rgb_net.params, self, 1)
        return sigmas

    @torch.no_grad()
    def _density_feat(self, x):
        n = x.shape[0]
        sigmas, _, enc, packed, _ = self._field_fwd(x, None, None, 1, True)
        h = torch.empty(n, 16, dtype=torch.float32, device=x.device)
        if n > 0:
            call("ncn_head_feat", enc, n, None, packed, self._prec, h)
        return sigmas, h

    def forward(self, x, d, **kwargs):
        x = x.float().contiguous()
        d = d.float().contiguous()
        _lib.check_input(x, "x")
        _lib.check_input(d, "d")
        n_dev = kwargs.get("n_samples_dev")
        if self._heads:
            sigmas, rgbs, *outs = _FieldHeadsFunction.apply(x, d, n_dev, self, *[p for p, _, _ in self._param_slices()])
            output = {"sigmas": sigmas, "rgbs": rgbs}
            for (name, _, _, _), o in zip(self._heads, outs):
                output["sems" if name == "sem_net" else "norms"] = o
            return output
        sigmas, rgbs = _FieldFunction.apply(x, d, self.xyz_encoder.params, self.sigma_net.params,
                                            self.rgb_net.params, self, 0, n_dev)
        return {"sigmas": sigmas, "rgbs": rgbs}

    @torch.no_grad()
    def get_all_cells(self):
        indices = vren.morton3D(self.grid_coords).long()
        return [(indices, self.grid_coords)] * self.cascades

    @torch.no_grad()
    def sample_uniform_and_occupied_cells(self, M, density_threshold):
        cells = []
        for c in range(self.cascades):
            coords1 = torch.randint(self.grid_size, (M, 3), dtype=torch.int32, device=self.density_grid.device)
            indices1 = vren.morton3D(coords1).long()
            indices2 = torch.nonzero(self.density_grid[c] > density_threshold)[:, 0]
            if len(indices2) > 0:
                rand_idx = torch.randint(len(indices2), (M,), device=self.density_grid.device)
                indices2 = indices2[rand_idx]
            coords2 = vren.morton3D_invert(indices2.int().contiguous())
            cells += [(torch.cat([indices1, indices2]), torch.cat([coords1, coords2]))]
        return cells

    @torch.no_grad()
    def mark_invisible_cells(self, K, dev, poses, img_wh, near_distance, chunk=64 ** 3):
        N_cams = poses.shape[0]
        self.count_grid = torch.zeros_like(self.density_grid)
        w2c_R = rearrange(poses[:, :3, :3], "n a b -> n b a")
        w2c_T = -w2c_R @ poses[:, :3, 3:]
        cells = self.get_all_cells()
        if isinstance(K, torch.Tensor):
            K = K.to(dev)
        elif isinstance(K, tuple):
            M_ndc_from_cam, M_uv_from_ndc = K[0].to(dev), K[1].to(dev)
            k_scale = K[3]
        else:
            raise AssertionError
        for c in range(self.cascades):
            indices, coords = cells[c]
            for i in range(0, len(indices), chunk):
                xyzs = coords[i:i + chunk] / (self.grid_size - 1) * 2 - 1
                s = min(2 ** (c - 1), self.scale)
                half_grid_size = s / self.grid_size
                xyzs_w = (xyzs * (s - half_grid_size)).T
                xyzs_c = w2c_R @ xyzs_w + w2c_T
                if isinstance(K, torch.Tensor):
                    uvd = K @ xyzs_c
                    uv = uvd[:, :2] / uvd[:, 2:]
                else:
                    xyzs_c *= 2 * k_scale
                    xyzs_c = torch.cat((xyzs_c, torch.ones_like(xyzs_c)[:, :1, :]), 1)
                    xyz_clip = M_ndc_from_cam @ xyzs_c
                    xyz_ndc = xyz_clip / xyz_clip[:, 3:]
                    uvd = M_uv_from_ndc @ xyz_ndc
                    uv = uvd[:, :2]
                in_image = (uvd[:, 2] >= 0) & (uv[:, 0] >= 0) & (uv[:, 0] < img_wh[0]) & (uv[:, 1] >= 0) & \
                           (uv[:, 1] < img_wh[1])
                covered_by_cam = (uvd[:, 2] >= near_distance) & in_image
                self.count_grid[c, indices[i:i + chunk]] = count = covered_by_cam.sum(0) / N_cams
                too_near_to_cam = (uvd[:, 2] < near_distance) & in_image
                valid_mask = (count > 0) & (~too_near_to_cam.any(0))
                self.density_grid[c, indices[i:i + chunk]] = torch.where(valid_mask, 0., -1.)

    def _grid_side_stream(self):
        if getattr(self, "_grid_side", None) is None:
            self._grid_side = torch.cuda.Stream(device=self.density_grid.device)
        return self._grid_side

    def _grid_ws(self):
        dev, N = self.density_grid.device, self.grid_size ** 3
        ws = getattr(self, "_gws", None)
        if ws is None or ws["xyzs"].device != dev or ws["idx"].numel() != N:
            nbytes = int(_lib.lib().ncn_grid_work_bytes())
            ws = {"xyzs": torch.empty(N, 3, device=dev), "idx": torch.empty(N, dtype=torch.int32, device=dev),
                  "sigmas": torch.empty(N, device=dev), "scal": torch.zeros(4, dtype=torch.int32, device=dev),
                  "enc": torch.empty(((N + 15) // 16) * 16 * ENC_BYTES // 2, dtype=torch.float16, device=dev),
                  "work": torch.zeros((nbytes + 15) // 16 * 4, dtype=torch.float32, device=dev)}
            self._gws = ws
        return ws

    @torch.no_grad()
    def update_density_grid(self, density_threshold, warmup=False, decay=0.95, erode=False, seed=None, beside=None):
        G, C = self.grid_size, self.cascades
        N = G ** 3
        dg = self.density_grid
        if not (dg.is_cuda and dg.is_contiguous() and dg.dtype == torch.float32 and dg.shape == (C, N)):
            raise RuntimeError("density_grid must be a contiguous CUDA float32 (cascades, grid_size**3) tensor")
        cnt = None
        if erode:
            cnt = self.count_grid.float().contiguous()
        ws = self._grid_ws()
        n_list = ws["scal"][0:1]
        if seed is None:
            seed = int(torch.randint(0, 2 ** 62, (1,)).item())
        table = self.xyz_encoder.params
        packed = None
        for c in range(C):
            s = min(2 ** (c - 1), self.scale)
            half_grid_size = s / G
            dgc = dg[c]
            cc = cnt[c] if cnt is not None else None

            def sample():
                call("ncn_grid_sample", dgc, N, G, s - half_grid_size, half_grid_size, density_threshold, N // 4,
                     1 if warmup else 0, (seed + 0x9E3779B97F4A7C15 * c) % 2 ** 64, decay, cc, ws["xyzs"], ws["idx"],
                     n_list, ws["work"])

            if c == 0 and beside is not None:
                cur = torch.cuda.current_stream(dg.device)
                side = self._grid_side_stream()
                side.wait_stream(cur)
                with torch.cuda.stream(side):
                    sample()
                beside()
                cur.wait_stream(side)
            else:
                sample()
            if packed is None:
                packed = self._take_packed()
            call("ncn_field_fwd", ws["xyzs"], None, N, n_list, None, table, self._levels_ptr, self._xyz_min,
                 self._xyz_extent, packed, self._prec, 2, ws["sigmas"], None, ws["enc"])
            call("ncn_grid_apply", dgc, ws["idx"], ws["sigmas"], n_list, N, decay, cc)
        thr_out = ws["scal"][1:2].view(torch.float32)
        call("ncn_grid_packbits", dg, C * N, density_threshold, self.density_bitfield, thr_out, ws["work"])


def register_grid_buffers(model):
    G = model.grid_size
    model.register_buffer("density_grid", torch.zeros(model.cascades, G ** 3, device=model.center.device))
    r = torch.arange(G, dtype=torch.int32, device=model.center.device)
    zz, yy, xx = torch.meshgrid(r, r, r, indexing="ij")
    coords = torch.stack([xx, yy, zz], -1).reshape(-1, 3)
    model.register_buffer("grid_coords", coords.contiguous())
    return model
```

normal-clustering-nerf_amd/ncnerf_amd/optim.py:

```python
import math

import torch

from . import _lib
from ._lib import call


def cosine_factor(epoch, num_epochs):
    return 0.5 * (1 + math.cos(math.pi * epoch / num_epochs))


POSE_LR = 1e-6


class PoseAdam:

    def __init__(self, params, lr=POSE_LR, betas=(0.9, 0.999), eps=1e-8):
        self.params = list(params)
        self.lr, self.betas, self.eps = lr, betas, eps
        self.m = [torch.zeros_like(p) for p in self.params]
        self.v = [torch.zeros_like(p) for p in self.params]
        self.t = torch.zeros((), dtype=torch.float64, device=self.params[0].device)

    def zero_grad(self):
        for p in self.params:
            p.grad = None

    def state_tensors(self):
        return self.params + self.m + self.v + [self.t]

    @torch.no_grad()
    def step(self, lr_factor=1.0):
        grads = [torch.zeros_like(p) if p.grad is None else p.grad for p in self.params]
        ok = torch.stack([torch.isfinite(g).all() for g in grads]).all()
        b1, b2 = self.betas
        t = self.t + 1
        c1, c2 = (1 - b1 ** t).float(), (1 - b2 ** t).float()
        for p, g, m, v in zip(self.params, grads, self.m, self.v):
            m_new = b1 * m + (1 - b1) * g
            v_new = b2 * v + (1 - b2) * g * g
            p_new = p - (self.lr * lr_factor) * (m_new / c1) / ((v_new / c2).sqrt() + self.eps)
            p.copy_(torch.where(ok, p_new, p))
            m.copy_(torch.where(ok, m_new, m))
            v.copy_(torch.where(ok, v_new, v))
        self.t.copy_(torch.where(ok, t, self.t))


class FlatAdam:
    def __init__(self, model, lr=1e-2, betas=(0.9, 0.999), eps=1e-15, weight_decay=(0.0, 1e-6), max_norm=0.05,
                 num_epochs=None, zero_grad_on_step=False):
        self.model = model
        self.base_lr = self.lr = lr
        self.betas, self.eps, self.wd, self.max_norm = betas, eps, weight_decay, max_norm
        flat = model.flat_params()
        self.m = torch.zeros_like(flat)
        self.v = torch.zeros_like(flat)
        self.part = torch.empty(1024, dtype=torch.float32, device=flat.device)
        self.work = torch.zeros(int(_lib.lib().ncn_adam_step_work_floats()), dtype=torch.float32, device=flat.device)
        self.step_count = 0
        self.step_dev = torch.zeros((), dtype=torch.int32, device=flat.device)
        self.lr_dev = torch.full((), float(lr), dtype=torch.float32, device=flat.device)
        self.num_epochs = num_epochs
        self.n_table = model._n_table
        self.zero_grad_on_step = zero_grad_on_step
        self.epoch = 0
        self.gate = torch.ones((), dtype=torch.int32, device=flat.device)
        self.pack_fused = hasattr(model, "pack_target") and not getattr(model, "_heads", None)
        if self.pack_fused:
            model.pack_target()

    def zero_grad(self):
        self.model.flat_grad().zero_()

    def set_epoch(self, epoch):
        if self.num_epochs and epoch != self.epoch:
            self.epoch = epoch
            self.lr = self.base_lr * cosine_factor(epoch, self.num_epochs)
            self.lr_dev.fill_(self.lr)

    def step(self, grad_scale=1.0, gated=False):
        self.step_count += 1
        p = self.model.flat_params()
        g = self.model.flat_grad()
        b1, b2 = self.betas
        args = [p, g, self.m, self.v, p.numel(), self.n_table, grad_scale, self.max_norm, self.lr, b1, b2, self.eps,
                self.wd[0], self.wd[1], self.lr_dev, self.step_dev, self.work, 1 if self.zero_grad_on_step else 0,
                getattr(self.model, "amp_state", None), self.gate if gated else None]
        if self.pack_fused:
            inv, off, packed, prec = self.model.pack_target()
            call("ncn_adam_step_packed", *args, inv, off, packed, prec)
            self.model._packed_fresh = True
        else:
            call("ncn_adam_step", *args)
            if getattr(self.model, "_heads", None):
                self.model.prepare_weights()

    def state_tensors(self):
        st = [self.model.flat_params(), self.m, self.v, self.step_dev, self.lr_dev]
        amp = getattr(self.model, "amp_state", None)
        return st + ([amp] if amp is not None else [])
```

normal-clustering-nerf_amd/ncnerf_amd/rendering.py:

```python
import time

import torch
from einops import rearrange

from .custom_functions import (CountJob, ExtraChannels, RayAABBIntersector, RayMarcher, VolumeRenderer,
                               VolumeRendererBg)
from . import _lib, vren


@torch.autocast("cuda")
def render(model, rays_o, rays_d, **kwargs):
    near_distance = kwargs["near_distance"]
    rays_o = rays_o.contiguous()
    rays_d = rays_d.contiguous()
    if (torch.is_grad_enabled() and (rays_o.requires_grad or rays_d.requires_grad)
            and not kwargs.get("test_time", False)):
        if kwargs.get("static_shapes", False) or kwargs.get("premarched") is not None:
            raise RuntimeError("render(): rays_o / rays_d require grad (pose refinement), which the static-shape / "
                               "premarched path cannot back-propagate: call render() without static_shapes")
    if kwargs.get("premarched") is not None and not kwargs.get("test_time", False):
        return render_rays_train(model, rays_o, rays_d, None, **kwargs)
    if _fused_march_ok(model, kwargs, rays_o.shape[0]):
        kwargs["premarched"] = march_train_fused(model, rays_o, rays_d, near_distance, kwargs["max_samples"],
                                                 kwargs.get("march_noise"), kwargs.get("march_rng"))
        return render_rays_train(model, rays_o, rays_d, None, **kwargs)
    _, hits_t, _ = vren.ray_aabb_intersect(rays_o.float(), rays_d.float(), model.center, model.half_size, 1,
                                           near_distance=near_distance)
    render_func = render_rays_test if kwargs.get("test_time", False) else render_rays_train
    results = render_func(model, rays_o, rays_d, hits_t, **kwargs)
    for k, v in results.items():
        if kwargs.get("to_cpu", False):
            v = v.cpu()
            if kwargs.get("to_numpy", False):
                v = v.numpy()
        results[k] = v
    return results


@torch.no_grad()
def render_rays_test(model, rays_o, rays_d, hits_t, **kwargs):
    exp_step_factor = kwargs.get("exp_step_factor", 0.0)
    max_samples = kwargs["max_samples"]
    results = {}
    N_rays = len(rays_o)
    device = rays_o.device
    opacity = torch.zeros(N_rays, device=device)
    depth = torch.zeros(N_rays, device=device)
    rend_l = 3 + (3 if model.pred_norm else 0) + (kwargs["n_sem_cls"] if model.pred_sem else 0)
    rend = torch.zeros(N_rays, rend_l, device=device)
    samples = total_samples = 0
    alive_indices = torch.arange(N_rays, device=device)
    min_samples = 1 if exp_step_factor == 0 else 4
    hits_t0 = hits_t[:, 0].contiguous()
    stats = kwargs.get("loop_stats")
    mode = kwargs.get("test_fused", True)
    fused = bool(mode) and not model.pred_norm and not model.pred_sem and hasattr(model, "_field_fwd")
    fwd_kwargs = {k: v for k, v in kwargs.items() if k not in ("loop_stats", "test_fused")}
    if fused and hasattr(model, "prepare_weights"):
        model.prepare_weights()
    if fused and mode is True and N_rays > 0:
        total_samples = _test_loop_device(model, rays_o, rays_d, hits_t0, alive_indices, exp_step_factor, max_samples,
                                          min_samples, float(kwargs.get("T_threshold", 1e-4)), opacity, depth, rend,
                                          stats)
        samples = max_samples
    while samples < max_samples:
        N_alive = len(alive_indices)
        if N_alive == 0:
            break
        N_samples = max(min(N_rays // N_alive, 64), min_samples)
        samples += N_samples
        xyzs, dirs, deltas, ts, N_eff_samples = vren.raymarching_test(
            rays_o, rays_d, hits_t0, alive_indices, model.density_bitfield, model.cascades, model.scale,
            exp_step_factor, model.grid_size, max_samples, N_samples)
        total_samples += N_eff_samples.sum()
        xyzs = rearrange(xyzs, "n1 n2 c -> (n1 n2) c")
        dirs = rearrange(dirs, "n1 n2 c -> (n1 n2) c")
        if fused:
            if stats is not None:
                stats["iterations"] = stats.get("iterations", 0) + 1
                stats["samples_marched"] = stats.get("samples_marched", 0) + N_alive * N_samples
            if hasattr(model, "prepare_weights"):
                model._packed_fresh = True
            cap = N_alive * N_samples
            xyz_c = torch.empty(cap, 3, dtype=torch.float32, device=device)
            dir_c = torch.empty(cap, 3, dtype=torch.float32, device=device)
            offs = torch.empty(N_alive, dtype=torch.int32, device=device)
            cnt = torch.empty(1, dtype=torch.int32, device=device)
            _lib.call("ncn_test_compact", xyzs, dirs, N_eff_samples, N_alive, N_samples, offs, xyz_c, dir_c, cnt)
            sig, rgb = model._field_fwd(xyz_c, dir_c, cnt, 0, False)[:2]
            _lib.call("ncn_composite_test_fw_compact", sig, rgb, offs, deltas, ts, alive_indices, N_alive, N_samples, 3,
                      float(kwargs.get("T_threshold", 1e-4)), N_eff_samples, opacity, depth, rend)
            if stats is not None:
                t0 = time.perf_counter()
            alive_indices = alive_indices[alive_indices >= 0]
            if stats is not None:
                stats["blocked_s"] = stats.get("blocked_s", 0.0) + time.perf_counter() - t0
            continue
        valid_mask = ~torch.all(dirs == 0, dim=1)
        if stats is not None:
            t0 = time.perf_counter()
        if valid_mask.sum() == 0:
            break
        if stats is not None:
            stats["blocked_s"] = stats.get("blocked_s", 0.0) + time.perf_counter() - t0
            stats["iterations"] = stats.get("iterations", 0) + 1
            stats["samples_marched"] = stats.get("samples_marched", 0) + N_alive * N_samples
        output = model(xyzs[valid_mask], dirs[valid_mask], **fwd_kwargs)
        sigmas = torch.zeros(len(xyzs), device=device)
        sigmas[valid_mask] = output["sigmas"].float()
        sigmas = rearrange(sigmas, "(n1 n2) -> n1 n2", n2=N_samples)
        rgbs = torch.zeros(len(xyzs), 3, device=device)
        rgbs[valid_mask] = output["rgbs"].float()
        raws = rearrange(rgbs, "(n1 n2) c -> n1 n2 c", n2=N_samples)
        for key in (("norms",) if model.pred_norm else ()) + (("sems",) if model.pred_sem else ()):
            extra = torch.zeros(len(xyzs), output[key].shape[1], device=device)
            extra[valid_mask] = output[key].float()
            raws = torch.cat((raws, rearrange(extra, "(n1 n2) c -> n1 n2 c", n2=N_samples)), dim=-1)
        vren.composite_test_multi_fw(sigmas.contiguous(), raws.contiguous(), deltas, ts, hits_t0, alive_indices,
                                     kwargs.get("T_threshold", 1e-4), N_eff_samples, opacity, depth, rend)
        if stats is not None:
            t0 = time.perf_counter()
        alive_indices = alive_indices[alive_indices >= 0]
        if stats is not None:
            stats["blocked_s"] += time.perf_counter() - t0
    hits_t[:, 0] = hits_t0
    results["opacity"] = opacity
    results["depth"] = depth
    i = 3
    results["rgb"] = rend[..., :i]
    if model.pred_norm:
        results["norm_nn"] = rend[..., i:i + 3]
        if kwargs.get("pred_norm_nn_norm", False):
            results["norm_nn"] = torch.nn.functional.normalize(results["norm_nn"], p=2.0, dim=-1)
        i += 3
    if model.pred_sem:
        results["sem"] = rend[..., i:i + kwargs["n_sem_cls"]]
    results["total_samples"] = total_samples
    rgb_bg = torch.ones(3, device=device) if exp_step_factor == 0 else torch.zeros(3, device=device)
    results["rgb"] += rgb_bg * rearrange(1 - opacity, "n -> n 1")
    return results


TEST_LOOP_CHECK = 4


def _test_loop_device(model, rays_o, rays_d, hits_t0, alive, exp_step_factor, max_samples, min_samples, T_threshold,
                      opacity, depth, rend, stats):
    from ._lib import call
    R, dev = rays_o.shape[0], rays_o.device
    cap = R * min_samples
    f = lambda *shape: torch.empty(*shape, dtype=torch.float32, device=dev)
    xyzs, dirs, deltas, ts = f(cap, 3), f(cap, 3), f(cap), f(cap)
    sig, rgb = f(cap), f(cap, 3)
    n_eff = torch.empty(R, dtype=torch.int32, device=dev)
    idx = torch.empty(cap, dtype=torch.int32, device=dev)
    model._packed_fresh = True
    packed = model._take_packed()
    bufs = [alive, torch.empty(R, dtype=torch.int64, device=dev)]
    ns0 = max(1, min_samples)
    ctrl = torch.tensor([R, ns0, ns0, 0, 0, 0, 0, 0], dtype=torch.int32, device=dev)
    total = torch.zeros(1, dtype=torch.int64, device=dev)
    count = ctrl[4:5]
    it = 0
    blocked = 0.0
    while it <= max_samples:
        for _ in range(TEST_LOOP_CHECK):
            a, b = bufs[it % 2], bufs[(it + 1) % 2]
            call("ncn_test_loop_march", rays_o, rays_d, hits_t0, a, R, model.density_bitfield,
                 int(model.cascades), float(model.scale), float(exp_step_factor), int(model.grid_size),
                 int(max_samples), ctrl, xyzs, dirs, deltas, ts, n_eff)
            call("ncn_test_loop_index", n_eff, R, ctrl, idx)
            call("ncn_field_fwd", xyzs, dirs, cap, count, idx, model.xyz_encoder.params, model._levels_ptr,
                 model._xyz_min, model._xyz_extent, packed, model._prec, 0, sig, rgb, None)
            call("ncn_test_loop_composite", sig, rgb, None, deltas, ts, a, R,
                 ctrl, 3, T_threshold, n_eff, opacity, depth, rend)
            call("ncn_test_loop_next", a, b, R, ctrl, total, R, int(max_samples), int(min_samples))
            it += 1
        t0 = time.perf_counter()
        done = bool(ctrl[3].item())
        blocked += time.perf_counter() - t0
        if done:
            break
    if stats is not None:
        c = ctrl.tolist()
        stats["iterations"] = stats.get("iterations", 0) + c[6]
        stats["samples_marched"] = stats.get("samples_marched", 0) + c[7]
        stats["blocked_s"] = stats.get("blocked_s", 0.0) + blocked
        stats["launched_iterations"] = stats.get("launched_iterations", 0) + it
    return total[0]


def render_rays_train(model, rays_o, rays_d, hits_t, **kwargs):
    exp_step_factor = kwargs.get("exp_step_factor", 0.0)
    max_samples = kwargs["max_samples"]
    results = {}
    anneal_step = kwargs.get("anneal_steps", 0)
    global_step = kwargs.get("global_step", anneal_step)
    if anneal_step > global_step:
        strategy = kwargs.get("anneal_strategy", "none")
        if strategy == "avoid_near":
            ps = 0.5
            ray_mid = (hits_t[:, 0, 0] + hits_t[:, 0, 1]) / 2.0
            n_i = min(max(global_step / anneal_step, ps), 1.0)
            hits_t[:, 0, 0] = ray_mid + n_i * (hits_t[:, 0, 0] - ray_mid)
        elif strategy == "depth":
            depth = kwargs["depth"]
            n_i = min(max(global_step / anneal_step, 0.05), 100.0)
            hits_t[:, 0, 0] = torch.max(depth + n_i * (hits_t[:, 0, 0] - depth), hits_t[:, 0, 0])
            hits_t[:, 0, 1] = torch.min(depth + n_i * (hits_t[:, 0, 1] - depth), hits_t[:, 0, 1])
        else:
            assert strategy == "none"
    if hasattr(model, "prepare_weights") and not getattr(model, "_packed_fresh", False):
        model.prepare_weights()
    static = bool(kwargs.get("static_shapes", False))
    pm = kwargs.get("premarched")
    if pm is not None:
        static = True
        rays_a, xyzs, dirs, results["deltas"], results["ts"], results["rm_samples"] = (
            pm["rays_a"], pm["xyzs"], pm["dirs"], pm["deltas"], pm["ts"], pm["counter"][0])
    else:
        rays_a, xyzs, dirs, results["deltas"], results["ts"], results["rm_samples"] = RayMarcher.apply(
            rays_o, rays_d, hits_t[:, 0], model.density_bitfield, model.cascades, model.scale, exp_step_factor,
            model.grid_size, max_samples, kwargs.get("march_noise"), static)
    for k, v in list(kwargs.items()):
        if isinstance(v, torch.Tensor) and k not in ("march_noise", "premarched", "march_rng", "count_acc"):
            if static:
                raise NotImplementedError(f"per-ray tensor kwarg {k!r} on the static-shape path")
            kwargs[k] = torch.repeat_interleave(v[rays_a[:, 0]], rays_a[:, 2], 0)
    if static:
        kwargs["n_samples_dev"] = results["rm_samples"]
    output = model(xyzs, dirs, **kwargs)
    sigmas = output["sigmas"]
    raws = output["rgbs"]
    extras = ([output["norms"]] if model.pred_norm else []) + ([output["sems"]] if model.pred_sem else [])
    fuse_bg = exp_step_factor == 0 and raws.shape[1] == 3
    renderer = VolumeRendererBg if fuse_bg else VolumeRenderer
    extra = (1.0,) if fuse_bg else ()
    job = CountJob() if fuse_bg and kwargs.get("count_in_loss") else None
    if fuse_bg and (kwargs.get("count_acc") is not None or job is not None):
        rm = results["rm_samples"]
        rm = rm if isinstance(rm, torch.Tensor) and rm.dtype == torch.int32 and rm.is_cuda else None
        acc = kwargs.get("count_acc")
        extra = (1.0, (rm if acc is not None else None, acc, job))
    (results["vr_samples"], results["opacity"], results["depth"], rend, results["ws"]) = renderer.apply(
        sigmas, raws.contiguous(), results["deltas"], results["ts"], rays_a, kwargs.get("T_threshold", 1e-4), *extra)
    if job is not None and job.out is not None:
        results["_count_job"] = job
    results["rgb"] = rend if rend.shape[-1] == 3 else rend[..., :3]
    if extras:
        rend_x = ExtraChannels.apply(results["ws"], extras[0] if len(extras) == 1 else torch.cat(extras, dim=-1), rays_a)
        i = 0
        if model.pred_norm:
            results["norm_nn"] = rend_x[..., :3]
            if kwargs.get("pred_norm_nn_norm", False):
                results["norm_nn"] = torch.nn.functional.normalize(results["norm_nn"], p=2.0, dim=-1)
            i = 3
        if model.pred_sem:
            results["sem"] = rend_x[..., i:i + kwargs["n_sem_cls"]]
    results["rays_d"] = rays_d
    results["rays_o"] = rays_d
    results["rays_a"] = rays_a
    results["depth_std"] = _ones(results["depth"])
    if exp_step_factor == 0:
        if not fuse_bg:
            results["rgb"] = results["rgb"] + (1 - results["opacity"])[:, None]
        return results
    if kwargs.get("random_bg", False):
        rgb_bg = torch.rand(3, device=rays_o.device)
    else:
        rgb_bg = torch.zeros(3, device=rays_o.device)
    results["rgb"] = results["rgb"] + rgb_bg * rearrange(1 - results["opacity"], "n -> n 1")
    return results


_ONES = {}


def _ones(like):
    key = (tuple(like.shape), like.dtype, like.device)
    t = _ONES.get(key)
    if t is None:
        t = _ONES[key] = torch.ones(like.shape, dtype=like.dtype, device=like.device)
    return t


def _fused_march_ok(model, kw, n_rays):
    return (kw.get("static_shapes", False) and not kw.get("test_time", False)
            and kw.get("exp_step_factor", 0.0) == 0 and kw.get("anneal_strategy", "none") == "none"
            and getattr(model, "_aabb", None) is not None and n_rays <= 16384
            and not any(isinstance(v, torch.Tensor) for k, v in kw.items()
                        if k not in ("march_noise", "march_rng", "count_acc")))


@torch.no_grad()
def march_train_fused(model, rays_o, rays_d, near_distance, max_samples, noise=None, rng=None, out=None):
    from ._lib import call, check_input, lib
    rays_o = rays_o.contiguous().float()
    rays_d = rays_d.contiguous().float()
    check_input(rays_o, "rays_o")
    check_input(rays_d, "rays_d")
    R, dev, ms = rays_o.shape[0], rays_o.device, int(max_samples)
    cap = R * ms
    if out is None:
        out = march_buffers(R, ms, dev)
    seed, ctr = 0, None
    if noise is not None:
        noise = noise.contiguous().float()
        check_input(noise, "noise")
    elif rng is not None:
        seed, ctr = rng
    else:
        noise = torch.rand_like(rays_o[:, 0])
    if out["xyzs"].shape[0] != cap or out["rays_a"].shape[0] != R:
        raise RuntimeError("march_train_fused: out= buffers are sized for another batch")
    slab_xyz, slab_t, slab_dt, ws = out["_slab"]
    c, h = model._aabb
    call("ncn_march_train_fused", rays_o, rays_d, R, c[0], c[1], c[2], h[0], h[1], h[2], near_distance, noise,
         int(seed) % 2 ** 64, ctr, model.density_bitfield, int(model.cascades), float(model.scale),
         int(model.grid_size), ms, slab_xyz, slab_t, slab_dt, ws, out["rays_a"], out["xyzs"], out["dirs"],
         out["deltas"], out["ts"], out["counter"])
    return out


def march_buffers(R, max_samples, device, share_scratch=None):
    from ._lib import lib
    cap = R * int(max_samples)
    f = lambda *shape: torch.empty(*shape, dtype=torch.float32, device=device)
    if share_scratch is not None:
        scratch = share_scratch["_slab"]
    else:
        ws = torch.empty((int(lib().ncn_march_train_fused_work_bytes(R)) + 3) // 4, dtype=torch.int32,
                         device=device)
        scratch = (f(cap * 3), f(cap), f(cap), ws)
    out = {"rays_a": torch.empty(R, 3, dtype=torch.int64, device=device), "xyzs": f(cap, 3), "dirs": f(cap, 3),
           "deltas": f(cap), "ts": f(cap), "counter": torch.empty(2, dtype=torch.int32, device=device),
           "_slab": scratch}
    return out



@torch.no_grad()
def march_train_static(model, rays_o, rays_d, out=None, **kwargs):
    exp_step_factor = kwargs.get("exp_step_factor", 0.0)
    rays_o = rays_o.contiguous().float()
    rays_d = rays_d.contiguous().float()
    _, hits_t, _ = vren.ray_aabb_intersect(rays_o, rays_d, model.center, model.half_size, 1,
                                           near_distance=kwargs["near_distance"])
    noise = kwargs.get("march_noise")
    if noise is None:
        noise = torch.rand_like(rays_o[:, 0])
    keys = ("rays_a", "xyzs", "dirs", "deltas", "ts", "counter")
    res = vren.raymarching_train(rays_o, rays_d, hits_t[:, 0].contiguous(), model.density_bitfield, model.cascades,
                                 model.scale, exp_step_factor, noise.contiguous(), model.grid_size,
                                 kwargs["max_samples"], static_capacity=True,
                                 out=None if out is None else [out[k] for k in keys])
    return dict(zip(keys, res))
```

normal-clustering-nerf_amd/ncnerf_amd/trainer.py:

```python
import math
import warnings

import torch

from . import _lib, distributed
from .losses import NeRFMTLoss, check_cluster_status
from .optim import POSE_LR, FlatAdam, PoseAdam, cosine_factor
from .rendering import march_train_fused, render

HYPERSIM_HPARAMS = dict(
    scale=0.5, grid_size=128, rend_max_samples=1024, rend_near_dist=0.01, density_tresh_decay=1.0,
    loss_opacity_w=1e-3, loss_distortion_w=0, loss_depth_w=0, loss_norm_depth_dot_w=0, loss_norm_depth_L1_w=0,
    loss_reg_depth_w=0, loss_sem_w=0, loss_manhattan_nerf_w=0,
    loss_norm_D_C_ort_dot_w=2e-3, loss_norm_D_C_centr_dot_w=2e-3, loss_norm_D_C_centr_L1_w=2e-3,
    loss_norm_D_C_can_dot_w=0, loss_norm_D_C_can_L1_w=0, loss_norm_can_tres=0.01, loss_norm_can_start=500,
    loss_norm_can_end=-1, loss_norm_can_grow=2500, lr=1e-2, num_epochs=30, batch_size=8192,
    ray_sampling_strategy="all_images_triang_patch", grad_clip=0.05, pred_norm_depth=True)

SCANNET_HPARAMS = dict(HYPERSIM_HPARAMS, loss_norm_D_C_ort_dot_w=1e-2, loss_norm_D_C_centr_dot_w=1e-2,
                       loss_norm_D_C_centr_L1_w=1e-2)

PRESETS = {"hypersim": HYPERSIM_HPARAMS, "scannet_manhattan": SCANNET_HPARAMS}


def hparams_for(preset):
    if preset not in PRESETS:
        raise ValueError(f"unknown preset {preset!r}; one of {sorted(PRESETS)}")
    return dict(PRESETS[preset])


_HOST_BATCH = "batch"


def rank_seed(dataset):
    return dataset.seed + distributed.rank()


def pose_lr(epoch, num_epochs):
    return POSE_LR * (cosine_factor(epoch, num_epochs) if num_epochs else 1.0)


class TrainLog:

    HEAD, TAIL = ("step", "total"), ("rm_samples", "vr_samples")

    def __init__(self, n_rays):
        self.n_rays = int(n_rays)
        self._segments = []

    @classmethod
    def column_names(cls, loss_d):
        return cls.HEAD + tuple(k for k in loss_d if k != "total") + cls.TAIL

    @staticmethod
    def ring_rows(first_step, count, capacity):
        if count > capacity:
            raise ValueError(f"{count} steps do not fit a ring of {capacity} rows: drained too late")
        return [(first_step + i) % capacity for i in range(count)]

    def add_ring(self, ring, columns, first_step, count):
        ring = torch.as_tensor(ring, dtype=torch.float32, device="cpu")
        if ring.dim() != 2 or ring.shape[1] != len(columns):
            raise ValueError(f"ring {tuple(ring.shape)} does not hold the {len(columns)} columns {tuple(columns)}")
        if count > 0:
            self._segments.append((tuple(columns), ring[self.ring_rows(first_step, count, ring.shape[0])].clone()))

    def __len__(self):
        return sum(rows.shape[0] for _, rows in self._segments)

    @property
    def columns(self):
        names = []
        for cols, _ in self._segments:
            names += [c for c in cols if c not in names]
        return tuple(names)

    def __getitem__(self, name):
        if name == "psnr":
            return -10.0 * torch.log10(self["rgb"])
        if name in ("rm_s", "vr_s"):
            return self[name[:2] + "_samples"] / float(self.n_rays)
        if name not in self.columns:
            raise KeyError(name)
        parts = [rows[:, cols.index(name)] if name in cols else torch.full((rows.shape[0],), float("nan"))
                 for cols, rows in self._segments]
        return torch.cat(parts) if parts else torch.empty(0)

    @property
    def steps(self):
        return self["step"].to(torch.int64) if self._segments else torch.empty(0, dtype=torch.int64)


class Trainer:
    warmup_steps = 256
    update_interval = 16

    epoch_items = 1000

    def __init__(self, model, hparams=None, update_grid=False, use_graph=False, scatter_split=None,
                 defer_optimizer=False, preset="hypersim", split_backward=True):
        self.h = dict(hparams_for(preset), **(hparams or {}))
        self.model = model
        self.loss = NeRFMTLoss(self.h)
        self.opt = FlatAdam(model, lr=self.h["lr"], max_norm=self.h["grad_clip"], num_epochs=self.h["num_epochs"],
                            zero_grad_on_step=True)
        self.world = distributed.world_size()
        self.steps_per_epoch = math.ceil(self.epoch_items / self.world)
        if self.world > 1:
            model.scatter_split = distributed.DEFAULT_SCATTER_SPLIT if scatter_split is None else scatter_split
        self.update_grid = update_grid
        self.render_kwargs = dict(near_distance=self.h["rend_near_dist"], max_samples=self.h["rend_max_samples"],
                                  test_time=False, random_bg=False, anneal_strategy="none", anneal_steps=0)
        if getattr(model, "pred_sem", False):
            self.render_kwargs["n_sem_cls"] = model.n_sem_cls
        if getattr(model, "pred_norm", False):
            self.render_kwargs["pred_norm_nn_norm"] = bool(self.h.get("pred_norm_nn_norm", False))
        self.use_graph = use_graph
        self.split_backward = bool(split_backward) and use_graph
        self.split_fused = split_backward != "forked"
        self._split = None
        self.graph = None
        self.defer = bool(defer_optimizer) and use_graph
        self._grad_scale = distributed.grad_scale_after_reduce(model, self.world)
        self._pending = False
        self._rng_seed = int(torch.randint(0, 2 ** 62, (1,)).item())
        self.grid_seed = None
        self.last_batch = None
        self._source = None
        self.pose_opt = None
        self._pose_ds = None
        self._log_ring = self._log_buf = self._log_cols = self._log_step = None
        self._log_capacity = self.log_capacity

    log_capacity = 1024

    def flush_optimizer(self):
        if self._pending:
            self.opt.step(grad_scale=self._grad_scale)
            self._pending = False

    def _maybe_update_grid(self, global_step):
        m = self.model
        if self.update_grid and global_step % self.update_interval == 0:
            thr = 0.01 * self.h["rend_max_samples"] / 3 ** 0.5 * self.h["density_tresh_decay"]
            seed = self.grid_seed(global_step) if self.grid_seed is not None else None
            m.update_density_grid(thr, warmup=global_step < self.warmup_steps, seed=seed, beside=self.flush_optimizer)
            distributed.broadcast_occupancy(m)

    def _body(self, batch, step_dev, with_opt):
        m = self.model
        if self._source is not _HOST_BATCH:
            batch = self._source.batch(step_dev, out=batch, seed=self._seed)
        kw = dict(self.render_kwargs, global_step=0, static_shapes=True)
        kw["count_in_loss"] = True
        if "march_noise" in batch:
            kw["march_noise"] = batch["march_noise"]
        else:
            kw["march_rng"] = (self._rng_seed, step_dev)
        if self.defer:
            cur = torch.cuda.current_stream()
            side = self._side_stream()
            side.wait_stream(cur)

            def optimizer():
                self.opt.step(gated=True, grad_scale=self._grad_scale)
                if not self.opt.pack_fused:
                    m._pack_weights()
                m._packed_fresh = True

            def marcher(out=None):
                return march_train_fused(m, batch["rays_o"], batch["rays_d"], kw["near_distance"], kw["max_samples"],
                                         kw.get("march_noise"), kw.get("march_rng"), out=out)

            with torch.cuda.stream(side):
                optimizer()
            kw["premarched"] = marcher()
            cur.wait_stream(side)
        if self._split is not None:
            results, loss_d = self._split.run(batch, step_dev, premarched=kw.get("premarched"))
        else:
            results = render(m, batch["rays_o"], batch["rays_d"], **kw)
            loss_d = self.loss(results, batch, global_step=step_dev)
            torch.autograd.backward(loss_d["total"], grad_tensors=self._unit(loss_d["total"].device))
        if with_opt and not self.defer:
            self.opt.step()
        if self._source is not _HOST_BATCH:
            self._log_row(results, loss_d, step_dev)
        return results, loss_d

    def _log_row(self, results, loss_d, step_dev):
        cols = TrainLog.column_names(loss_d)
        if self._log_ring is None or cols != self._log_cols:
            f = dict(dtype=torch.float32, device=step_dev.device)
            self._log_ring, self._log_buf, self._log_cols = torch.zeros(self._log_capacity, len(cols), **f), torch.zeros(
                len(cols), **f), cols
        with torch.no_grad():
            row, n = self._log_buf, len(cols)
            torch.stack([loss_d["total"]] + [loss_d[k] for k in cols[2:-2]], out=row[1:n - 2])
            row[0].copy_(step_dev)
            row[n - 2].copy_(results["rm_samples"])
            row[n - 1].copy_(results["vr_samples"])
            at = torch.remainder(step_dev, self._log_ring.shape[0]).reshape(1)
            self._log_ring.index_copy_(0, at, row.reshape(1, n))

    def _unit(self, dev):
        if getattr(self, "_one", None) is None or self._one.device != dev:
            self._one = torch.ones((), dtype=torch.float32, device=dev)
        return self._one

    def _side_stream(self):
        if getattr(self, "_side", None) is None:
            self._side = torch.cuda.Stream(device=self.model.flat_params().device)
        return self._side

    def _capture(self, batch, dataset=None):
        if self.render_kwargs.get("anneal_steps", 0) > 0:
            raise NotImplementedError("ray-range annealing is step-dependent host control flow")
        if dataset is not None:
            dev = dataset.device
            self._static = dict(dataset.buffers(), patch_area=dataset.patch_size * dataset.patch_size,
                                x1_offsets_local=dataset.x1_off, x2_offsets_local=dataset.x2_off,
                                x3_offsets_local=dataset.x3_off)
            self._seed = rank_seed(dataset)
        else:
            dev = batch["rays_o"].device
            self._static = {k: (v.clone() if isinstance(v, torch.Tensor) else v) for k, v in batch.items()}
        self._source = _HOST_BATCH if dataset is None else dataset
        from .split_step import SplitStep, split_eligible
        self._split = None
        if self.split_backward and split_eligible(self, self._static):
            try:
                self._split = SplitStep(self, fused=self.split_fused)
            except _lib.NcnError as e:
                warnings.warn(f"split backward unavailable on this device, using the autograd step: {e}")
        self._step_dev = torch.zeros((), dtype=torch.int64, device=dev)
        self._with_opt = not distributed.is_distributed() and self.model.scatter_split is None
        state = self.opt.state_tensors()
        saved = [t.clone() for t in state]
        saved_count = self.opt.step_count
        side = torch.cuda.Stream(device=dev)
        side.wait_stream(torch.cuda.current_stream(dev))
        with torch.cuda.stream(side):
            for _ in range(2):
                self._body(self._static, self._step_dev, self._with_opt)
        torch.cuda.current_stream(dev).wait_stream(side)
        self.model._deferred = []
        self.model._packed_fresh = False
        self.graph = torch.cuda.CUDAGraph()
        import gc
        gc.collect()
        gc_was_on = gc.isenabled()
        gc.disable()
        try:
            with torch.cuda.graph(self.graph):
                self._out = self._body(self._static, self._step_dev, self._with_opt)
        finally:
            if gc_was_on:
                gc.enable()
        self.model._deferred_graph = self.model._deferred
        self.model._deferred = []
        for t, v in zip(state, saved):
            t.copy_(v)
        if hasattr(self.model, "prepare_weights"):
            self.model.prepare_weights()
        self.opt.step_count = saved_count
        self.model.flat_grad().zero_()

    def _graph_step(self, batch, global_step, dataset=None):
        if self.graph is None:
            self._capture(batch, dataset)
        self.last_batch = self._static
        dst, src = [], []
        for k, v in ({} if batch is None else batch).items():
            if k in self._static and hasattr(v, "copy_") and v is not self._static[k]:
                dst.append(self._static[k])
                src.append(v)
        fast = len(dst) <= 8 and all(
            s.is_cuda and s.is_contiguous() and d.is_contiguous() and s.dtype == d.dtype and s.shape == d.shape
            for s, d in zip(src, dst))
        gate = 1 if self._pending else 0
        if fast:
            _lib.step_inputs(src, dst, self._step_dev, global_step, self.opt.gate if self.defer else None, gate)
        else:
            if dst:
                torch._foreach_copy_(dst, src, non_blocking=True)
            self._step_dev.fill_(global_step)
            if self.defer:
                self.opt.gate.fill_(gate)
        self.graph.replay()
        scale = distributed.reduce_gradients(self.model, graph=True) if not self._with_opt else 1.0
        if self.defer:
            self.opt.step_count += gate
            self._pending = True
        elif not self._with_opt:
            self.opt.step(grad_scale=scale)
        else:
            self.opt.step_count += 1
        return self._out

    status_interval = 100

    def _check_source(self, dataset):
        if not self.use_graph:
            return
        if dataset is not None and dataset.optimize_ext:
            raise NotImplementedError(
                "Trainer(use_graph=True) cannot refine the poses of a dataset with optimize_ext: the captured step "
                "renders with static shapes, and that render refuses rays that require grad (rendering.render; "
                "RayMarcher.backward has no static-capacity ray gradient).  Use Trainer(use_graph=False).")
        want = _HOST_BATCH if dataset is None else dataset
        if self._source is None or self._source is want:
            return
        have = ("a host-built batch (step())" if self._source is _HOST_BATCH
                else "the DeviceRayDataset of its first step_from(): the draw is part of the graph")
        raise RuntimeError(f"the captured step takes its batch from {have}; it cannot train on "
                           f"{'a host-built batch' if dataset is None else 'another source'}.  "
                           "Use one Trainer per source.")

    def _prologue(self, global_step):
        if global_step % self.status_interval == 0:
            check_cluster_status(self.model.flat_params().device)
        self._maybe_update_grid(global_step)
        epoch = global_step // self.steps_per_epoch
        if epoch != self.opt.epoch:
            self.flush_optimizer()
        self.opt.set_epoch(epoch)

    def _eager_step(self, batch, global_step):
        m = self.model
        self.last_batch = batch
        kw = dict(self.render_kwargs, global_step=global_step)
        if "march_noise" in batch:
            kw["march_noise"] = batch["march_noise"]
        results = render(m, batch["rays_o"], batch["rays_d"], **kw)
        loss_d = self.loss(results, batch, global_step=global_step)
        loss_d["total"].backward()
        self.opt.step(grad_scale=distributed.reduce_gradients(m))
        return results, loss_d

    def step(self, batch, global_step):
        self._check_source(None)
        self._prologue(global_step)
        if self.use_graph:
            return self._graph_step(batch, global_step)
        return self._eager_step(batch, global_step)

    def step_from(self, dataset, global_step):
        self._check_source(dataset)
        pose = None
        if dataset.optimize_ext:
            if self.world > 1:
                raise NotImplementedError("pose refinement is single-process: the pose gradients are not all-reduced")
            if self._pose_ds is not dataset:
                self.pose_opt, self._pose_ds = PoseAdam([dataset.dR, dataset.dT]), dataset
            pose = self.pose_opt
        self._prologue(global_step)
        if self.use_graph:
            return self._graph_step(None, global_step, dataset)
        if pose is not None:
            pose.zero_grad()
        out = self._eager_step(dataset.batch(global_step, seed=rank_seed(dataset)), global_step)
        if pose is not None:
            pose.step(cosine_factor(self.opt.epoch, self.h["num_epochs"]) if self.h.get("num_epochs") else 1.0)
        return out

    def fit(self, dataset, n_steps, start_step=0, callback=None, callback_every=0, log_capacity=None):
        n_steps, start_step = int(n_steps), int(start_step)
        capacity = n_steps if log_capacity is None else int(log_capacity)
        if n_steps < 1 or capacity < 1:
            raise ValueError(f"fit: n_steps {n_steps} and log_capacity {capacity} must be at least 1")
        self._check_source(dataset)
        if self.graph is None:
            self._log_capacity = capacity
            self._log_ring = None
        log = TrainLog(dataset.batch_size)
        first = start_step
        for s in range(start_step, start_step + n_steps):
            results, loss_d = self.step_from(dataset, s)
            if not self.use_graph:
                if self._log_step is None:
                    self._log_step = torch.zeros((), dtype=torch.int64, device=dataset.device)
                self._log_step.fill_(s)
                cols = TrainLog.column_names(loss_d)
                if self._log_ring is not None and cols != self._log_cols and s > first:
                    self._drain(log, first, s - first)
                    first = s
                self._log_row(results, loss_d, self._log_step)
            if s + 1 - first == min(capacity, self._log_ring.shape[0]):
                self._drain(log, first, s + 1 - first)
                first = s + 1
            if callback is not None and callback_every > 0 and (s + 1) % callback_every == 0:
                self.flush_optimizer()
                callback(self, s)
        self.flush_optimizer()
        self._drain(log, first, start_step + n_steps - first)
        return log

    def _drain(self, log, first_step, count):
        if count > 0:
            log.add_ring(self._log_ring.cpu(), self._log_cols, first_step, count)
```

Baseline: 12.17 million rays/s.

## Fuse deferred Adam apply into ray-march walk/place kernels via block role split

Adds a fused front kernel pair in which some workgroups run the ray-march walk and place phases while the remaining workgroups apply the deferred Adam update over a split of the parameter range. This replaces the previous two-stream fork, where the optimizer ran on a side stream concurrently with the marcher, with a single stream. The goal is to remove stream fork/join and separate kernel launches while keeping both workloads co-resident on the GPU. The risk is contention between march and optimizer blocks within one grid, plus a waves-per-EU occupancy hint that may constrain register allocation.

```diff
diff --git a/normal-clustering-nerf_amd/csrc/front_fused.hip b/normal-clustering-nerf_amd/csrc/front_fused.hip
--- /dev/null
+++ b/normal-clustering-nerf_amd/csrc/front_fused.hip
@@ -0,0 +1,191 @@
+#pragma clang fp contract(off)
+#include <algorithm>
+#include "common.h"
+#include "../../include/ncnerf.h"
+#include "ncnerf_front.h"
+#include "vren_march.h"
+#include "vren_march_wave.h"
+#include "vren_march_pack.h"
+#pragma clang fp contract(fast)
+#include "optim_apply.h"
+#pragma clang fp contract(off)
+
+namespace ncn {
+
+__device__ __forceinline__ bool front_role(unsigned b, unsigned A, unsigned F, unsigned& idx) {
+    if (b >= F) {
+        idx = b - A;
+        return false;
+    }
+    const unsigned f0 = b * A / F, f1 = (b + 1u) * A / F;
+    const bool marcher = f1 > f0;
+    idx = marcher ? f0 : b - f0;
+    return marcher;
+}
+
+struct FrontAdam {
+    float *p, *g, *m, *v;
+    int64_t n, n0;
+    float b1, b2, eps, wd0, wd1;
+    const float* sc;
+    const int32_t* pinv;
+    int64_t poff;
+    void* packed;
+    int64_t lo, hi;
+};
+struct FrontWalk {
+    const float *rays_o, *rays_d;
+    int64_t R;
+    float cx, cy, cz, hx, hy, hz, near_distance;
+    const float* noise;
+    uint64_t seed;
+    const int64_t* rng_ctr;
+    const uint8_t* bitfield;
+    int cascades;
+    float scale;
+    int G, max_samples;
+    float *slab_xyz, *slab_t, *slab_dt;
+    int32_t *counts, *wg_sum;
+};
+struct FrontPlace {
+    const float* rays_d;
+    int64_t R;
+    int max_samples;
+    const int32_t *counts, *wg_sum;
+    const float *slab_xyz, *slab_t, *slab_dt;
+    int64_t* rays_a;
+    float *xyzs, *dirs, *deltas, *ts;
+    int32_t* counter;
+};
+
+template <bool ZERO, int PK>
+__device__ __forceinline__ void front_apply(unsigned wg, unsigned nwg, const FrontAdam& a) {
+    adam_apply_body<ZERO, PK, true>(RoleGrid{wg, nwg}, a.lo, a.hi, a.p, a.g, a.m, a.v, a.n, a.n0, a.b1, a.b2, a.eps,
+                                    a.wd0, a.wd1, a.sc, a.pinv, a.poff, a.packed);
+}
+
+#ifndef NCN_FRONT_WAVES
+#define NCN_FRONT_WAVES 5
+#endif
+#if NCN_FRONT_WAVES
+#define NCN_FRONT_BOUNDS __launch_bounds__(256) __attribute__((amdgpu_waves_per_eu(NCN_FRONT_WAVES)))
+#else
+#define NCN_FRONT_BOUNDS __launch_bounds__(256)
+#endif
+
+template <bool ONE_CASCADE, bool ZERO, int PK>
+__global__ NCN_FRONT_BOUNDS void front_walk_kernel(const FrontWalk w, const FrontAdam a, unsigned n_march,
+                                                   unsigned n_span) {
+    unsigned idx;
+    if (front_role(blockIdx.x, n_march, n_span, idx))
+        march_train_walk2_body<ONE_CASCADE, 2>(idx, w.rays_o, w.rays_d, w.R, w.cx, w.cy, w.cz, w.hx, w.hy, w.hz,
+                                               w.near_distance, w.noise, w.seed, w.rng_ctr, w.bitfield, w.cascades,
+                                               w.scale, w.G, w.max_samples, w.slab_xyz, w.slab_t, w.slab_dt, w.counts,
+                                               w.wg_sum);
+    else
+        front_apply<ZERO, PK>(idx, gridDim.x - n_march, a);
+}
+
+template <bool ZERO, int PK>
+__global__ NCN_FRONT_BOUNDS void front_place_kernel(const FrontPlace q, const FrontAdam a, unsigned n_march,
+                                                    unsigned n_span) {
+    unsigned idx;
+    if (front_role(blockIdx.x, n_march, n_span, idx))
+        march_train_place_body((int)idx, (int)n_march, q.rays_d, q.R, q.max_samples, q.counts, q.wg_sum, q.slab_xyz,
+                               q.slab_t, q.slab_dt, q.rays_a, q.xyzs, q.dirs, q.deltas, q.ts, q.counter);
+    else
+        front_apply<ZERO, PK>(idx, gridDim.x - n_march, a);
+}
+
+template <bool ONE_CASCADE, bool ZERO, int PK>
+static void launch_walk(int grid, hipStream_t s, const FrontWalk& w, const FrontAdam& a, unsigned n_march,
+                        unsigned n_span) {
+    hipLaunchKernelGGL((front_walk_kernel<ONE_CASCADE, ZERO, PK>), dim3(grid), dim3(256), 0, s, w, a, n_march, n_span);
+}
+template <bool ZERO, int PK>
+static void launch_place(int grid, hipStream_t s, const FrontPlace& q, const FrontAdam& a, unsigned n_march,
+                         unsigned n_span) {
+    hipLaunchKernelGGL((front_place_kernel<ZERO, PK>), dim3(grid), dim3(256), 0, s, q, a, n_march, n_span);
+}
+
+#ifndef NCN_FRONT_SPLIT_64THS
+#define NCN_FRONT_SPLIT_64THS 64
+#endif
+#ifndef NCN_FRONT_WALK_SPAN_8THS
+#define NCN_FRONT_WALK_SPAN_8THS 24
+#endif
+#ifndef NCN_FRONT_PLACE_SPAN_8THS
+#define NCN_FRONT_PLACE_SPAN_8THS 0
+#endif
+static unsigned front_span(int64_t n_march, int64_t grid, int eighths) {
+    return (unsigned)(eighths <= 0 ? grid : std::min<int64_t>(grid, std::max<int64_t>(n_march, n_march * eighths / 8)));
+}
+static int64_t front_default_split(int64_t n) { return n <= 0 ? 0 : (n / 64 * NCN_FRONT_SPLIT_64THS) & ~(int64_t)3; }
+
+}
+
+using namespace ncn;
+
+extern "C" {
+
+int64_t ncn_step_front_default_split(int64_t n) { return front_default_split(n); }
+
+int ncn_step_front(float* params, float* grads, float* exp_avg, float* exp_avg_sq, int64_t n, int64_t n_group0,
+                   float grad_scale, float max_norm, float lr, double beta1, double beta2, float eps, float wd0,
+                   float wd1, const float* lr_dev, int* step_dev, float* work, int zero_grads, float* amp_state,
+                   const int* gate, const int32_t* pack_inv, int64_t pack_off, uint16_t* packed, int pack_prec,
+                   const float* rays_o, const float* rays_d, int64_t n_rays, float cx, float cy, float cz, float hx,
+                   float hy, float hz, float near_distance, const float* noise, uint64_t seed,
+                   const int64_t* rng_counter, const uint8_t* bitfield, int cascades, float scale, int grid_size,
+                   int max_samples, float* slab_xyz, float* slab_t, float* slab_dt, void* march_work, int64_t* rays_a,
+                   float* xyzs, float* dirs, float* deltas, float* ts, int32_t* counter, int64_t adam_split,
+                   void* stream) {
+    if (const int rc = adam_pack_args_check("ncn_step_front", n, pack_inv, pack_off, packed, pack_prec)) return rc;
+    if (adam_split == -1) adam_split = front_default_split(n);
+    NCN_REQUIRE(adam_split >= 0 && adam_split <= n && (adam_split % 4 == 0 || adam_split == n), hipErrorInvalidValue,
+                "ncn_step_front: adam_split=%lld must be a multiple of 4 in [0, n] (or n, or -1 for the default)",
+                (long long)adam_split);
+    const int64_t nwg = n_rays > 0 ? cdiv(n_rays, 4) : 0;
+    if (n_rays > 0) {
+        NCN_REQUIRE(cascades >= 1 && grid_size >= 1 && grid_size <= 1024 && max_samples >= 1 && march_work != nullptr,
+                    hipErrorInvalidValue, "ncn_step_front: bad cascades/grid_size/max_samples/march_work");
+        NCN_REQUIRE(nwg <= PLACE_MAX_WG && n_rays * (int64_t)max_samples < (1ll << 31) && max_samples < (1 << 24),
+                    hipErrorInvalidValue, "ncn_step_front: n_rays must be <= %d (and n_rays * max_samples < 2^31)",
+                    4 * PLACE_MAX_WG);
+    }
+    const hipStream_t s = (hipStream_t)stream;
+    const float* sc = nullptr;
+    if (const int rc = adam_prep_launch("ncn_step_front", params, grads, exp_avg, exp_avg_sq, n, grad_scale, max_norm, lr,
+                                        beta1, beta2, lr_dev, step_dev, work, amp_state, gate, s, &sc))
+        return rc;
+    int32_t* counts = (int32_t*)march_work;
+    int32_t* wg_sum = counts + std::max<int64_t>(n_rays, 0);
+    const FrontWalk w = {rays_o, rays_d, n_rays, cx, cy, cz, hx, hy, hz, near_distance, noise, seed, rng_counter,
+                         bitfield, cascades, scale, grid_size, max_samples, slab_xyz, slab_t, slab_dt, counts, wg_sum};
+    const FrontPlace q = {rays_d, n_rays, max_samples, counts, wg_sum, slab_xyz, slab_t, slab_dt, rays_a,
+                          xyzs, dirs, deltas, ts, counter};
+    FrontAdam a = {params, grads, exp_avg, exp_avg_sq, n, n_group0, (float)beta1, (float)beta2, eps, wd0, wd1, sc,
+                   pack_inv, pack_off, packed, 0, adam_split};
+    const bool one = cascades == 1, zero = zero_grads != 0, f16 = pack_prec == NCN_PREC_F16;
+    const int grid1 = (int)nwg + adam_apply_blocks(adam_split);
+    if (grid1 > 0) {
+        const auto launch = one ? (zero ? (f16 ? launch_walk<true, true, 1> : launch_walk<true, true, 2>)
+                                        : (f16 ? launch_walk<true, false, 1> : launch_walk<true, false, 2>))
+                                : (zero ? (f16 ? launch_walk<false, true, 1> : launch_walk<false, true, 2>)
+                                        : (f16 ? launch_walk<false, false, 1> : launch_walk<false, false, 2>));
+        launch(grid1, s, w, a, (unsigned)nwg, front_span(nwg, grid1, NCN_FRONT_WALK_SPAN_8THS));
+        NCN_LAUNCH_CHECK("ncn_step_front (walk, apply)");
+    }
+    a.lo = adam_split;
+    a.hi = n;
+    const int grid2 = (int)nwg + adam_apply_blocks(n - adam_split);
+    if (grid2 > 0) {
+        const auto launch = zero ? (f16 ? launch_place<true, 1> : launch_place<true, 2>)
+                                 : (f16 ? launch_place<false, 1> : launch_place<false, 2>);
+        launch(grid2, s, q, a, (unsigned)nwg, front_span(nwg, grid2, NCN_FRONT_PLACE_SPAN_8THS));
+        NCN_LAUNCH_CHECK("ncn_step_front (place, apply)");
+    }
+    return 0;
+}
+
+}
diff --git a/normal-clustering-nerf_amd/csrc/ncnerf_front.h b/normal-clustering-nerf_amd/csrc/ncnerf_front.h
--- /dev/null
+++ b/normal-clustering-nerf_amd/csrc/ncnerf_front.h
@@ -0,0 +1,24 @@
+#ifndef NCNERF_FRONT_H
+#define NCNERF_FRONT_H
+#include <stdint.h>
+
+#ifdef __cplusplus
+extern "C" {
+#endif
+
+int ncn_step_front(float* params, float* grads, float* exp_avg, float* exp_avg_sq, int64_t n, int64_t n_group0,
+                   float grad_scale, float max_norm, float lr, double beta1, double beta2, float eps, float wd0,
+                   float wd1, const float* lr_dev, int* step_dev, float* work, int zero_grads, float* amp_state,
+                   const int* gate, const int32_t* pack_inv, int64_t pack_off, uint16_t* packed, int pack_prec,
+                   const float* rays_o, const float* rays_d, int64_t n_rays, float cx, float cy, float cz, float hx,
+                   float hy, float hz, float near_distance, const float* noise, uint64_t seed,
+                   const int64_t* rng_counter, const uint8_t* bitfield, int cascades, float scale, int grid_size,
+                   int max_samples, float* slab_xyz, float* slab_t, float* slab_dt, void* march_work, int64_t* rays_a,
+                   float* xyzs, float* dirs, float* deltas, float* ts, int32_t* counter, int64_t adam_split,
+                   void* stream);
+int64_t ncn_step_front_default_split(int64_t n);
+
+#ifdef __cplusplus
+}
+#endif
+#endif
diff --git a/normal-clustering-nerf_amd/csrc/optim.hip b/normal-clustering-nerf_amd/csrc/optim.hip
--- a/normal-clustering-nerf_amd/csrc/optim.hip
+++ b/normal-clustering-nerf_amd/csrc/optim.hip
@@ -1,5 +1,6 @@
 #include <algorithm>
 #include "workgroup.h"
+#include "optim_apply.h"
 #include "../../include/ncnerf.h"
 
 namespace ncn {
@@ -144,22 +145,6 @@
         }
     }
 }
-template <int PK>
-__device__ __forceinline__ void adam_pack1(int64_t e, float x, const int32_t* __restrict__ pinv, int64_t poff,
-                                           int64_t n, void* __restrict__ packed) {
-    if (PK == 0 || e < poff || e >= n) return;
-    const int64_t w = e - poff;
-    const int2 q = ((const int2*)pinv)[w];
-    if (PK == 1) {
-        const _Float16 h = (_Float16)x;
-        if (q.x >= 0) ((_Float16*)packed)[q.x] = h;
-        if (q.y >= 0) ((_Float16*)packed)[q.y] = h;
-    } else {
-        const __bf16 h = (__bf16)x;
-        if (q.x >= 0) ((__bf16*)packed)[q.x] = h;
-        if (q.y >= 0) ((__bf16*)packed)[q.y] = h;
-    }
-}
 template <bool ZERO, int PK>
 __global__ __launch_bounds__(256) void adam_apply_kernel(float* __restrict__ p, float* __restrict__ g,
                                                          float* __restrict__ m, float* __restrict__ v, int64_t n,
@@ -167,61 +152,8 @@
                                                          float wd1, const float* __restrict__ sc,
                                                          const int32_t* __restrict__ pinv, int64_t poff,
                                                          void* __restrict__ packed) {
-    const float cf = sc[0], bc1 = sc[1], bc2 = sc[2], lr = sc[3];
-    if (sc[4] != 0.f) {
-        if (PK) {
-            const int64_t tid = (int64_t)blockIdx.x * 256 + threadIdx.x, nth = (int64_t)gridDim.x * 256;
-            for (int64_t e = poff + tid; e < n; e += nth) adam_pack1<PK>(e, p[e], pinv, poff, n, packed);
-        }
-        if (ZERO) {
-            const int64_t tid = (int64_t)blockIdx.x * 256 + threadIdx.x, nth = (int64_t)gridDim.x * 256;
-            for (int64_t i = tid; i < n / 4; i += nth) ((float4*)g)[i] = make_float4(0.f, 0.f, 0.f, 0.f);
-            for (int64_t i = 4 * (n / 4) + tid; i < n; i += nth) g[i] = 0.f;
-        }
-        return;
-    }
-    auto upd = [&](float& pi, float gr, float& mi, float& vi, float wd) {
-        const float gi = gr * cf;
-        mi = b1 * mi + (1.f - b1) * gi;
-        vi = b2 * vi + (1.f - b2) * gi * gi;
-        const float denom = sqrtf(vi / bc2) + eps;
-        pi = pi - lr * ((mi / bc1) / denom + wd * pi);
-    };
-    auto upd_tail = [&](float& pi, float gr, float& mi, float& vi, float wd) {
-#pragma clang fp contract(off)
-        const float gi = gr * cf;
-        mi = fmaf(b1, mi, (1.f - b1) * gi);
-        vi = fmaf(b2, vi, ((1.f - b2) * gi) * gi);
-        const float denom = sqrtf(vi / bc2) + eps;
-        pi = fmaf(-lr, fmaf(wd, pi, (mi / bc1) / denom), pi);
-    };
-    const int64_t n4 = n / 4, tid = (int64_t)blockIdx.x * 256 + threadIdx.x, nth = (int64_t)gridDim.x * 256;
-#pragma unroll 2
-    for (int64_t i = tid; i < n4; i += nth) {
-        float4 P = ((float4*)p)[i], M = ((float4*)m)[i], V = ((float4*)v)[i];
-        const float4 G = ((const float4*)g)[i];
-        const int64_t e = 4 * i;
-        upd(P.x, G.x, M.x, V.x, e < n0 ? wd0 : wd1);
-        upd(P.y, G.y, M.y, V.y, e + 1 < n0 ? wd0 : wd1);
-        upd(P.z, G.z, M.z, V.z, e + 2 < n0 ? wd0 : wd1);
-        upd(P.w, G.w, M.w, V.w, e + 3 < n0 ? wd0 : wd1);
-        ((float4*)p)[i] = P;
-        ((float4*)m)[i] = M;
-        ((float4*)v)[i] = V;
-        if (PK && e + 3 >= poff) {
-            adam_pack1<PK>(e, P.x, pinv, poff, n, packed);
-            adam_pack1<PK>(e + 1, P.y, pinv, poff, n, packed);
-            adam_pack1<PK>(e + 2, P.z, pinv, poff, n, packed);
-            adam_pack1<PK>(e + 3, P.w, pinv, poff, n, packed);
-        }
-        if (ZERO && (G.x != 0.f || G.y != 0.f || G.z != 0.f || G.w != 0.f))
-            ((float4*)g)[i] = make_float4(0.f, 0.f, 0.f, 0.f);
-    }
-    for (int64_t i = 4 * n4 + tid; i < n; i += nth) {
-        upd_tail(p[i], g[i], m[i], v[i], i < n0 ? wd0 : wd1);
-        adam_pack1<PK>(i, p[i], pinv, poff, n, packed);
-        if (ZERO) g[i] = 0.f;
-    }
+    adam_apply_body<ZERO, PK, false>(LaunchGrid{}, 0, n, p, g, m, v, n, n0, b1, b2, eps, wd0, wd1, sc,
+                                     pinv, poff, packed);
 }
 constexpr int NCN_STEP_MAX_BUFS = 8;
 struct StepCopies {
@@ -342,6 +274,31 @@
 
 }
 
+int ncn::adam_prep_launch(const char* who, const float* params, const float* grads, const float* exp_avg,
+                          const float* exp_avg_sq, int64_t n, float grad_scale, float max_norm, float lr, double beta1,
+                          double beta2, const float* lr_dev, int* step_dev, float* work, float* amp_state,
+                          const int* gate, hipStream_t stream, const float** sc) {
+    NCN_REQUIRE(((((uintptr_t)params) | ((uintptr_t)grads) | ((uintptr_t)exp_avg) | ((uintptr_t)exp_avg_sq)) & 15) == 0,
+                hipErrorInvalidValue, "%s: buffers must be 16-byte aligned", who);
+    NCN_REQUIRE(step_dev != nullptr && work != nullptr, hipErrorInvalidValue,
+                "%s: needs the device step counter and the work buffer", who);
+    const int prep_blocks = (int)std::min<int64_t>(ADAM_BLOCKS, std::max<int64_t>(1, cdiv(n / 4, ADAM_THREADS * 4)));
+    hipLaunchKernelGGL(adam_prep_kernel, dim3(prep_blocks), dim3(ADAM_THREADS), 0, stream, grads, n, grad_scale,
+                       max_norm, beta1, beta2, lr, lr_dev, step_dev, work, amp_state, gate);
+    hipError_t e = hipGetLastError();
+    NCN_REQUIRE(e == hipSuccess, e, "%s (prep): launch failed: %s", who, hipGetErrorString(e));
+    *sc = work + ADAM_BLOCKS + 4;
+    return 0;
+}
+
+int ncn::adam_pack_args_check(const char* who, int64_t n, const int32_t* pack_inv, int64_t pack_off, const void* packed,
+                              int pack_prec) {
+    NCN_REQUIRE(pack_inv && packed && (pack_prec == NCN_PREC_F16 || pack_prec == NCN_PREC_BF16) && pack_off >= 0 &&
+                    n - pack_off == NCN_FIELD_NW && (((uintptr_t)pack_inv) & 7) == 0,
+                hipErrorInvalidValue, "%s: pack_inv/packed/pack_prec/pack_off invalid", who);
+    return 0;
+}
+
 template <int PK>
 static void launch_apply(int zero, int blocks, hipStream_t st, float* params, float* grads, float* exp_avg,
                          float* exp_avg_sq, int64_t n, int64_t n_group0, double beta1, double beta2, float eps,
@@ -360,17 +317,12 @@
                           float* amp_state, const int* gate, const int32_t* pinv, int64_t poff, void* packed, int pk,
                           void* stream) {
     if (n <= 0) return 0;
-    NCN_REQUIRE(((((uintptr_t)params) | ((uintptr_t)grads) | ((uintptr_t)exp_avg) | ((uintptr_t)exp_avg_sq)) & 15) == 0,
-                hipErrorInvalidValue, "ncn_adam_step: buffers must be 16-byte aligned");
-    NCN_REQUIRE(step_dev != nullptr && work != nullptr, hipErrorInvalidValue,
-                "ncn_adam_step: needs the device step counter and the work buffer");
-    const int prep_blocks = (int)std::min<int64_t>(ADAM_BLOCKS, std::max<int64_t>(1, cdiv(n / 4, ADAM_THREADS * 4)));
-    hipLaunchKernelGGL(adam_prep_kernel, dim3(prep_blocks), dim3(ADAM_THREADS), 0, (hipStream_t)stream, grads, n,
-                       grad_scale, max_norm, beta1, beta2, lr, lr_dev, step_dev, work, amp_state, gate);
-    NCN_LAUNCH_CHECK("ncn_adam_step (prep)");
-    const int blocks = (int)std::min<int64_t>(std::max<int64_t>(1, cdiv(n, 2048)), 16384);
-    const float* sc = work + ADAM_BLOCKS + 4;
     const hipStream_t st = (hipStream_t)stream;
+    const float* sc = nullptr;
+    if (const int rc = adam_prep_launch("ncn_adam_step", params, grads, exp_avg, exp_avg_sq, n, grad_scale, max_norm, lr,
+                                        beta1, beta2, lr_dev, step_dev, work, amp_state, gate, st, &sc))
+        return rc;
+    const int blocks = adam_apply_blocks(n);
     if (pk == 0)
         launch_apply<0>(zero_grads, blocks, st, params, grads, exp_avg, exp_avg_sq, n, n_group0, beta1, beta2, eps, wd0,
                         wd1, sc, nullptr, 0, nullptr);
@@ -399,9 +351,7 @@
                          float wd1, const float* lr_dev, int* step_dev, float* work, int zero_grads, float* amp_state,
                          const int* gate, const int32_t* pack_inv, int64_t pack_off, uint16_t* packed, int pack_prec,
                          void* stream) {
-    NCN_REQUIRE(pack_inv && packed && (pack_prec == NCN_PREC_F16 || pack_prec == NCN_PREC_BF16) && pack_off >= 0 &&
-                    n - pack_off == NCN_FIELD_NW && (((uintptr_t)pack_inv) & 7) == 0,
-                hipErrorInvalidValue, "ncn_adam_step_packed: pack_inv/packed/pack_prec/pack_off invalid");
+    if (const int rc = adam_pack_args_check("ncn_adam_step_packed", n, pack_inv, pack_off, packed, pack_prec)) return rc;
     return adam_step_impl(params, grads, exp_avg, exp_avg_sq, n, n_group0, grad_scale, max_norm, lr, beta1, beta2, eps,
                           wd0, wd1, lr_dev, step_dev, work, zero_grads, amp_state, gate, pack_inv, pack_off, packed,
                           pack_prec == NCN_PREC_F16 ? 1 : 2, stream);
diff --git a/normal-clustering-nerf_amd/csrc/optim_apply.h b/normal-clustering-nerf_amd/csrc/optim_apply.h
--- /dev/null
+++ b/normal-clustering-nerf_amd/csrc/optim_apply.h
@@ -0,0 +1,114 @@
+#pragma once
+#include "common.h"
+
+namespace ncn {
+
+template <int PK>
+__device__ __forceinline__ void adam_pack1(int64_t e, float x, const int32_t* __restrict__ pinv, int64_t poff,
+                                           int64_t n, void* __restrict__ packed) {
+    if (PK == 0 || e < poff || e >= n) return;
+    const int64_t w = e - poff;
+    const int2 q = ((const int2*)pinv)[w];
+    if (PK == 1) {
+        const _Float16 h = (_Float16)x;
+        if (q.x >= 0) ((_Float16*)packed)[q.x] = h;
+        if (q.y >= 0) ((_Float16*)packed)[q.y] = h;
+    } else {
+        const __bf16 h = (__bf16)x;
+        if (q.x >= 0) ((__bf16*)packed)[q.x] = h;
+        if (q.y >= 0) ((__bf16*)packed)[q.y] = h;
+    }
+}
+
+struct LaunchGrid {
+    __device__ __forceinline__ unsigned wg() const { return blockIdx.x; }
+    __device__ __forceinline__ unsigned nwg() const { return gridDim.x; }
+};
+struct RoleGrid {
+    unsigned wg_, nwg_;
+    __device__ __forceinline__ unsigned wg() const { return wg_; }
+    __device__ __forceinline__ unsigned nwg() const { return nwg_; }
+};
+
+template <bool ZERO, int PK, bool RANGED, typename Grid>
+__device__ __forceinline__ void adam_apply_body(const Grid grid, int64_t lo, int64_t hi, float* __restrict__ p,
+                                                float* __restrict__ g, float* __restrict__ m,
+                                                float* __restrict__ v, int64_t n, int64_t n0, float b1, float b2,
+                                                float eps, float wd0, float wd1, const float* __restrict__ sc,
+                                                const int32_t* __restrict__ pinv, int64_t poff,
+                                                void* __restrict__ packed) {
+    if (!RANGED) {
+        lo = 0;
+        hi = n;
+    }
+    const float cf = sc[0], bc1 = sc[1], bc2 = sc[2], lr = sc[3];
+    if (sc[4] != 0.f) {
+        if (PK) {
+            const int64_t tid = (int64_t)grid.wg() * 256 + threadIdx.x, nth = (int64_t)grid.nwg() * 256;
+            const int64_t e0 = RANGED ? (lo > poff ? lo : poff) : poff;
+            for (int64_t e = e0 + tid; e < hi; e += nth) adam_pack1<PK>(e, p[e], pinv, poff, n, packed);
+        }
+        if (ZERO) {
+            const int64_t tid = (int64_t)grid.wg() * 256 + threadIdx.x, nth = (int64_t)grid.nwg() * 256;
+            for (int64_t i = (RANGED ? lo / 4 : 0) + tid; i < hi / 4; i += nth)
+                ((float4*)g)[i] = make_float4(0.f, 0.f, 0.f, 0.f);
+            for (int64_t i = (RANGED && lo > 4 * (n / 4) ? lo : 4 * (n / 4)) + tid; i < hi; i += nth) g[i] = 0.f;
+        }
+        return;
+    }
+    auto upd = [&](float& pi, float gr, float& mi, float& vi, float wd) {
+        const float gi = gr * cf;
+        mi = b1 * mi + (1.f - b1) * gi;
+        vi = b2 * vi + (1.f - b2) * gi * gi;
+        const float denom = sqrtf(vi / bc2) + eps;
+        pi = pi - lr * ((mi / bc1) / denom + wd * pi);
+    };
+    auto upd_tail = [&](float& pi, float gr, float& mi, float& vi, float wd) {
+#pragma clang fp contract(off)
+        const float gi = gr * cf;
+        mi = fmaf(b1, mi, (1.f - b1) * gi);
+        vi = fmaf(b2, vi, ((1.f - b2) * gi) * gi);
+        const float denom = sqrtf(vi / bc2) + eps;
+        pi = fmaf(-lr, fmaf(wd, pi, (mi / bc1) / denom), pi);
+    };
+    const int64_t n4 = hi / 4, tid = (int64_t)grid.wg() * 256 + threadIdx.x, nth = (int64_t)grid.nwg() * 256;
+#pragma unroll 2
+    for (int64_t i = (RANGED ? lo / 4 : 0) + tid; i < n4; i += nth) {
+        float4 P = ((float4*)p)[i], M = ((float4*)m)[i], V = ((float4*)v)[i];
+        const float4 G = ((const float4*)g)[i];
+        const int64_t e = 4 * i;
+        upd(P.x, G.x, M.x, V.x, e < n0 ? wd0 : wd1);
+        upd(P.y, G.y, M.y, V.y, e + 1 < n0 ? wd0 : wd1);
+        upd(P.z, G.z, M.z, V.z, e + 2 < n0 ? wd0 : wd1);
+        upd(P.w, G.w, M.w, V.w, e + 3 < n0 ? wd0 : wd1);
+        ((float4*)p)[i] = P;
+        ((float4*)m)[i] = M;
+        ((float4*)v)[i] = V;
+        if (PK && e + 3 >= poff) {
+            adam_pack1<PK>(e, P.x, pinv, poff, n, packed);
+            adam_pack1<PK>(e + 1, P.y, pinv, poff, n, packed);
+            adam_pack1<PK>(e + 2, P.z, pinv, poff, n, packed);
+            adam_pack1<PK>(e + 3, P.w, pinv, poff, n, packed);
+        }
+        if (ZERO && (G.x != 0.f || G.y != 0.f || G.z != 0.f || G.w != 0.f))
+            ((float4*)g)[i] = make_float4(0.f, 0.f, 0.f, 0.f);
+    }
+    for (int64_t i = (RANGED && lo > 4 * (n / 4) ? lo : 4 * n4) + tid; i < hi; i += nth) {
+        upd_tail(p[i], g[i], m[i], v[i], i < n0 ? wd0 : wd1);
+        adam_pack1<PK>(i, p[i], pinv, poff, n, packed);
+        if (ZERO) g[i] = 0.f;
+    }
+}
+
+static inline int adam_apply_blocks(int64_t count) {
+    return count <= 0 ? 0 : (int)(cdiv(count, 2048) < 16384 ? cdiv(count, 2048) : 16384);
+}
+
+int adam_prep_launch(const char* who, const float* params, const float* grads, const float* exp_avg,
+                     const float* exp_avg_sq, int64_t n, float grad_scale, float max_norm, float lr, double beta1,
+                     double beta2, const float* lr_dev, int* step_dev, float* work, float* amp_state, const int* gate,
+                     hipStream_t stream, const float** sc);
+int adam_pack_args_check(const char* who, int64_t n, const int32_t* pack_inv, int64_t pack_off, const void* packed,
+                         int pack_prec);
+
+}
diff --git a/normal-clustering-nerf_amd/csrc/vren_march_pack.h b/normal-clustering-nerf_amd/csrc/vren_march_pack.h
--- a/normal-clustering-nerf_amd/csrc/vren_march_pack.h
+++ b/normal-clustering-nerf_amd/csrc/vren_march_pack.h
@@ -4,7 +4,7 @@
 
 namespace ncn {
 
-__global__ __launch_bounds__(1024) void march_train_scan_kernel(const int32_t* __restrict__ counts, int64_t R,
+inline __global__ __launch_bounds__(1024) void march_train_scan_kernel(const int32_t* __restrict__ counts, int64_t R,
                                                                 int64_t* __restrict__ rays_a,
                                                                 int32_t* __restrict__ counter) {
     __shared__ int wave_tot[16];
@@ -52,7 +52,7 @@
     }
 }
 
-__global__ __launch_bounds__(256) void march_train_pack_kernel(
+inline __global__ __launch_bounds__(256) void march_train_pack_kernel(
     const float* __restrict__ rays_d, const int64_t* __restrict__ rays_a, int64_t R, int max_samples,
     const float* __restrict__ slab_xyz, const float* __restrict__ slab_t, const float* __restrict__ slab_dt,
     float* __restrict__ xyzs, float* __restrict__ dirs, float* __restrict__ deltas, float* __restrict__ ts) {
@@ -66,19 +66,19 @@
                   slab_dt + ray * (int64_t)max_samples, d3, 0, cnt, start, lane, xyzs, dirs, deltas, ts);
 }
 
-__global__ __launch_bounds__(256) void march_train_place_kernel(
-    const float* __restrict__ rays_d, int64_t R, int max_samples, const int32_t* __restrict__ counts,
-    const int32_t* __restrict__ wg_sum, const float* __restrict__ slab_xyz, const float* __restrict__ slab_t,
-    const float* __restrict__ slab_dt, int64_t* __restrict__ rays_a, float* __restrict__ xyzs,
-    float* __restrict__ dirs, float* __restrict__ deltas, float* __restrict__ ts, int32_t* __restrict__ counter) {
+__device__ __forceinline__ void march_train_place_body(
+    const int b, const int nwg, const float* __restrict__ rays_d, int64_t R, int max_samples,
+    const int32_t* __restrict__ counts, const int32_t* __restrict__ wg_sum, const float* __restrict__ slab_xyz,
+    const float* __restrict__ slab_t, const float* __restrict__ slab_dt, int64_t* __restrict__ rays_a,
+    float* __restrict__ xyzs, float* __restrict__ dirs, float* __restrict__ deltas, float* __restrict__ ts,
+    int32_t* __restrict__ counter) {
     __shared__ int red[4][3];
     const int lane = threadIdx.x & 63, wv = threadIdx.x >> 6;
-    const int b = blockIdx.x;
     int v[PLACE_MAX_WG / 256];
 #pragma unroll
     for (int u = 0; u < PLACE_MAX_WG / 256; u++) {
         const int i = u * 256 + threadIdx.x;
-        v[u] = i < (int)gridDim.x ? wg_sum[i] : 0;
+        v[u] = i < nwg ? wg_sum[i] : 0;
     }
     const int64_t r0 = __builtin_amdgcn_readfirstlane((int)(b * 4 + wv));
     const bool live = r0 < R;
@@ -122,7 +122,7 @@
     }
     const int64_t row = n > PLACE_LONG ? (int64_t)(long_before + lw)
                                        : (int64_t)long_total + (4 * (int64_t)b - long_before) + (wv - lw);
-    if (b == (int)gridDim.x - 1 && threadIdx.x == 0) {
+    if (b == nwg - 1 && threadIdx.x == 0) {
         counter[0] = start + len[0] + len[1] + len[2] + len[3];
         counter[1] = (int32_t)R;
     }
@@ -153,4 +153,13 @@
     copy_slab_row(sx, st, sd, d3, PF * 64, n, start, lane, xyzs, dirs, deltas, ts);
 }
 
+inline __global__ __launch_bounds__(256) void march_train_place_kernel(
+    const float* __restrict__ rays_d, int64_t R, int max_samples, const int32_t* __restrict__ counts,
+    const int32_t* __restrict__ wg_sum, const float* __restrict__ slab_xyz, const float* __restrict__ slab_t,
+    const float* __restrict__ slab_dt, int64_t* __restrict__ rays_a, float* __restrict__ xyzs,
+    float* __restrict__ dirs, float* __restrict__ deltas, float* __restrict__ ts, int32_t* __restrict__ counter) {
+    march_train_place_body((int)blockIdx.x, (int)gridDim.x, rays_d, R, max_samples, counts, wg_sum, slab_xyz, slab_t,
+                           slab_dt, rays_a, xyzs, dirs, deltas, ts, counter);
 }
+
+}
diff --git a/normal-clustering-nerf_amd/csrc/vren_march_wave.h b/normal-clustering-nerf_amd/csrc/vren_march_wave.h
--- a/normal-clustering-nerf_amd/csrc/vren_march_wave.h
+++ b/normal-clustering-nerf_amd/csrc/vren_march_wave.h
@@ -217,15 +217,15 @@
 constexpr int PLACE_LONG = 256;
 
 template <bool ONE_CASCADE, int P>
-__global__ __launch_bounds__(256) void march_train_walk2_kernel(
-    const float* __restrict__ rays_o, const float* __restrict__ rays_d, int64_t R, float cx, float cy, float cz,
-    float hx, float hy, float hz, float near_distance, const float* __restrict__ noise, uint64_t seed,
+__device__ __forceinline__ void march_train_walk2_body(
+    const unsigned wg, const float* __restrict__ rays_o, const float* __restrict__ rays_d, int64_t R, float cx, float cy,
+    float cz, float hx, float hy, float hz, float near_distance, const float* __restrict__ noise, uint64_t seed,
     const int64_t* __restrict__ rng_ctr, const uint8_t* __restrict__ bitfield, int cascades, float scale, int G,
     int max_samples, float* __restrict__ slab_xyz, float* __restrict__ slab_t, float* __restrict__ slab_dt,
     int32_t* __restrict__ counts, int32_t* __restrict__ wg_sum) {
     __shared__ int cnt_s[4];
     const int lane = threadIdx.x & 63, wv = threadIdx.x >> 6;
-    const int64_t r0 = __builtin_amdgcn_readfirstlane((int)(blockIdx.x * 4 + wv));
+    const int64_t r0 = __builtin_amdgcn_readfirstlane((int)(wg * 4 + wv));
     const bool live = r0 < R;
     const int64_t r = live ? r0 : R - 1;
     const MarchConst m = make_march_const(cascades, scale, 0.0f, G, max_samples, scale);
@@ -254,8 +254,20 @@
         int nl = 0;
 #pragma unroll
         for (int w = 0; w < 4; w++) nl += cnt_s[w] > PLACE_LONG;
-        wg_sum[blockIdx.x] = (cnt_s[0] + cnt_s[1] + cnt_s[2] + cnt_s[3]) | (nl << 26);
-    }
-}
-
-}
+        wg_sum[wg] = (cnt_s[0] + cnt_s[1] + cnt_s[2] + cnt_s[3]) | (nl << 26);
+    }
+}
+
+template <bool ONE_CASCADE, int P>
+__global__ __launch_bounds__(256) void march_train_walk2_kernel(
+    const float* __restrict__ rays_o, const float* __restrict__ rays_d, int64_t R, float cx, float cy, float cz,
+    float hx, float hy, float hz, float near_distance, const float* __restrict__ noise, uint64_t seed,
+    const int64_t* __restrict__ rng_ctr, const uint8_t* __restrict__ bitfield, int cascades, float scale, int G,
+    int max_samples, float* __restrict__ slab_xyz, float* __restrict__ slab_t, float* __restrict__ slab_dt,
+    int32_t* __restrict__ counts, int32_t* __restrict__ wg_sum) {
+    march_train_walk2_body<ONE_CASCADE, P>(blockIdx.x, rays_o, rays_d, R, cx, cy, cz, hx, hy, hz, near_distance, noise,
+                                           seed, rng_ctr, bitfield, cascades, scale, G, max_samples, slab_xyz, slab_t,
+                                           slab_dt, counts, wg_sum);
+}
+
+}
diff --git a/normal-clustering-nerf_amd/ncnerf_amd/_lib.py b/normal-clustering-nerf_amd/ncnerf_amd/_lib.py
--- a/normal-clustering-nerf_amd/ncnerf_amd/_lib.py
+++ b/normal-clustering-nerf_amd/ncnerf_amd/_lib.py
@@ -130,10 +130,25 @@
 
 ABI, HEADER_OF, CONSTANTS, NON_LITERAL_DEFINES = load_headers()
 AMP_INIT_SCALE = CONSTANTS["NCN_AMP_INIT_SCALE"]
+INTERNAL_HEADER = os.path.join(os.path.dirname(_HERE), "csrc", "ncnerf_front.h")
+
+
+def load_internal(path=INTERNAL_HEADER, public=ABI):
+    try:
+        decls = parse_header(open(path).read())
+    except OSError as e:
+        raise NcnError(f"{path} not found: the binding of the step's fused front is derived from it ({e})") from None
+    for name in decls:
+        if name in public:
+            raise NcnError(f"{name} is declared in {os.path.basename(path)} and in include/{HEADER_OF.get(name)}")
+    return decls
+
+
+INTERNAL_ABI = load_internal()
 
 
 def declaration(name):
-    return ABI[name]
+    return ABI[name] if name in ABI else INTERNAL_ABI[name]
 
 
 def symbols(header=None):
@@ -162,9 +177,12 @@
             raise NcnError(f"libncnerf.so not found at {LIB_PATH}: run __graft_entry__.build() "
                            f"(make -C normal-clustering-nerf_amd)")
         L = ctypes.CDLL(LIB_PATH)
-        for name, (ret, _) in ABI.items():
-            fn = getattr(L, name)
-            fn.argtypes = SIGNATURES[name]
+        for name, (ret, params) in (*ABI.items(), *INTERNAL_ABI.items()):
+            try:
+                fn = getattr(L, name)
+            except AttributeError:
+                raise NcnError(f"{LIB_PATH} does not export {name}: rebuild it (make -C normal-clustering-nerf_amd)") from None
+            fn.argtypes = [P if kind == "ptr" else _SCALARS[kind] for kind, _, _ in params]
             fn.restype = _RESTYPES[ret]
         _lib = L
     return _lib
@@ -227,7 +245,7 @@
     return ns["marshal"], (n - 1, n) if _launches(params) else (n,)
 
 
-_PLANS = {name: _marshaller(name, params) for name, (_, params) in ABI.items()}
+_PLANS = {name: _marshaller(name, params) for name, (_, params) in (*ABI.items(), *INTERNAL_ABI.items())}
 
 
 def marshal(name, args):
diff --git a/normal-clustering-nerf_amd/ncnerf_amd/ngp_mt.py b/normal-clustering-nerf_amd/ncnerf_amd/ngp_mt.py
--- a/normal-clustering-nerf_amd/ncnerf_amd/ngp_mt.py
+++ b/normal-clustering-nerf_amd/ncnerf_amd/ngp_mt.py
@@ -508,6 +508,15 @@
             self._grid_side = torch.cuda.Stream(device=self.density_grid.device)
         return self._grid_side
 
+    def open_grid_side_stream(self):
+        cur = torch.cuda.current_stream(self.density_grid.device)
+        side = self._grid_side_stream()
+        t = torch.empty(1, device=self.density_grid.device)
+        side.wait_stream(cur)
+        with torch.cuda.stream(side):
+            t.zero_()
+        cur.wait_stream(side)
+
     def _grid_ws(self):
         dev, N = self.density_grid.device, self.grid_size ** 3
         ws = getattr(self, "_gws", None)
diff --git a/normal-clustering-nerf_amd/ncnerf_amd/optim.py b/normal-clustering-nerf_amd/ncnerf_amd/optim.py
--- a/normal-clustering-nerf_amd/ncnerf_amd/optim.py
+++ b/normal-clustering-nerf_amd/ncnerf_amd/optim.py
@@ -78,14 +78,25 @@
             self.lr = self.base_lr * cosine_factor(epoch, self.num_epochs)
             self.lr_dev.fill_(self.lr)
 
-    def step(self, grad_scale=1.0, gated=False):
-        self.step_count += 1
+    def _step_args(self, grad_scale, gated):
         p = self.model.flat_params()
         g = self.model.flat_grad()
         b1, b2 = self.betas
-        args = [p, g, self.m, self.v, p.numel(), self.n_table, grad_scale, self.max_norm, self.lr, b1, b2, self.eps,
+        return [p, g, self.m, self.v, p.numel(), self.n_table, grad_scale, self.max_norm, self.lr, b1, b2, self.eps,
                 self.wd[0], self.wd[1], self.lr_dev, self.step_dev, self.work, 1 if self.zero_grad_on_step else 0,
                 getattr(self.model, "amp_state", None), self.gate if gated else None]
+
+    def step_front(self, march_args, grad_scale=1.0, gated=False, adam_split=-1):
+        if not self.pack_fused:
+            raise RuntimeError("step_front: the model's optimizer step does not write the packed fragments")
+        self.step_count += 1
+        inv, off, packed, prec = self.model.pack_target()
+        call("ncn_step_front", *self._step_args(grad_scale, gated), inv, off, packed, prec, *march_args, int(adam_split))
+        self.model._packed_fresh = True
+
+    def step(self, grad_scale=1.0, gated=False):
+        self.step_count += 1
+        args = self._step_args(grad_scale, gated)
         if self.pack_fused:
             inv, off, packed, prec = self.model.pack_target()
             call("ncn_adam_step_packed", *args, inv, off, packed, prec)
diff --git a/normal-clustering-nerf_amd/ncnerf_amd/rendering.py b/normal-clustering-nerf_amd/ncnerf_amd/rendering.py
--- a/normal-clustering-nerf_amd/ncnerf_amd/rendering.py
+++ b/normal-clustering-nerf_amd/ncnerf_amd/rendering.py
@@ -292,9 +292,8 @@
                         if k not in ("march_noise", "march_rng", "count_acc")))
 
 
-@torch.no_grad()
-def march_train_fused(model, rays_o, rays_d, near_distance, max_samples, noise=None, rng=None, out=None):
-    from ._lib import call, check_input, lib
+def march_train_fused_args(model, rays_o, rays_d, near_distance, max_samples, noise=None, rng=None, out=None):
+    from ._lib import check_input
     rays_o = rays_o.contiguous().float()
     rays_d = rays_d.contiguous().float()
     check_input(rays_o, "rays_o")
@@ -315,10 +314,17 @@
         raise RuntimeError("march_train_fused: out= buffers are sized for another batch")
     slab_xyz, slab_t, slab_dt, ws = out["_slab"]
     c, h = model._aabb
-    call("ncn_march_train_fused", rays_o, rays_d, R, c[0], c[1], c[2], h[0], h[1], h[2], near_distance, noise,
-         int(seed) % 2 ** 64, ctr, model.density_bitfield, int(model.cascades), float(model.scale),
-         int(model.grid_size), ms, slab_xyz, slab_t, slab_dt, ws, out["rays_a"], out["xyzs"], out["dirs"],
-         out["deltas"], out["ts"], out["counter"])
+    args = [rays_o, rays_d, R, c[0], c[1], c[2], h[0], h[1], h[2], near_distance, noise, int(seed) % 2 ** 64, ctr,
+            model.density_bitfield, int(model.cascades), float(model.scale), int(model.grid_size), ms, slab_xyz, slab_t,
+            slab_dt, ws, out["rays_a"], out["xyzs"], out["dirs"], out["deltas"], out["ts"], out["counter"]]
+    return args, out
+
+
+@torch.no_grad()
+def march_train_fused(model, rays_o, rays_d, near_distance, max_samples, noise=None, rng=None, out=None):
+    from ._lib import call
+    args, out = march_train_fused_args(model, rays_o, rays_d, near_distance, max_samples, noise, rng, out)
+    call("ncn_march_train_fused", *args)
     return out
 
 
diff --git a/normal-clustering-nerf_amd/ncnerf_amd/trainer.py b/normal-clustering-nerf_amd/ncnerf_amd/trainer.py
--- a/normal-clustering-nerf_amd/ncnerf_amd/trainer.py
+++ b/normal-clustering-nerf_amd/ncnerf_amd/trainer.py
@@ -6,7 +6,7 @@
 from . import _lib, distributed
 from .losses import NeRFMTLoss, check_cluster_status
 from .optim import POSE_LR, FlatAdam, PoseAdam, cosine_factor
-from .rendering import march_train_fused, render
+from .rendering import march_train_fused, march_train_fused_args, render
 
 HYPERSIM_HPARAMS = dict(
     scale=0.5, grid_size=128, rend_max_samples=1024, rend_near_dist=0.01, density_tresh_decay=1.0,
@@ -98,7 +98,9 @@
     epoch_items = 1000
 
     def __init__(self, model, hparams=None, update_grid=False, use_graph=False, scatter_split=None,
-                 defer_optimizer=False, preset="hypersim", split_backward=True):
+                 defer_optimizer=False, preset="hypersim", split_backward=True, front="fused"):
+        if front not in ("fused", "forked"):
+            raise ValueError(f"front must be 'fused' or 'forked', got {front!r}")
         self.h = dict(hparams_for(preset), **(hparams or {}))
         self.model = model
         self.loss = NeRFMTLoss(self.h)
@@ -121,6 +123,7 @@
         self._split = None
         self.graph = None
         self.defer = bool(defer_optimizer) and use_graph
+        self.front_fused = front == "fused" and self.opt.pack_fused
         self._grad_scale = distributed.grad_scale_after_reduce(model, self.world)
         self._pending = False
         self._rng_seed = int(torch.randint(0, 2 ** 62, (1,)).item())
@@ -157,7 +160,12 @@
             kw["march_noise"] = batch["march_noise"]
         else:
             kw["march_rng"] = (self._rng_seed, step_dev)
-        if self.defer:
+        if self.defer and self.front_fused:
+            args, kw["premarched"] = march_train_fused_args(m, batch["rays_o"], batch["rays_d"], kw["near_distance"],
+                                                            kw["max_samples"], kw.get("march_noise"), kw.get("march_rng"))
+            self.opt.step_front(args, gated=True, grad_scale=self._grad_scale)
+            m._packed_fresh = True
+        elif self.defer:
             cur = torch.cuda.current_stream()
             side = self._side_stream()
             side.wait_stream(cur)
@@ -234,6 +242,8 @@
             except _lib.NcnError as e:
                 warnings.warn(f"split backward unavailable on this device, using the autograd step: {e}")
         self._step_dev = torch.zeros((), dtype=torch.int64, device=dev)
+        if self.update_grid and self.defer and hasattr(self.model, "open_grid_side_stream"):
+            self.model.open_grid_side_stream()
         self._with_opt = not distributed.is_distributed() and self.model.scatter_split is None
         state = self.opt.state_tensors()
         saved = [t.clone() for t in state]
```

Measured after the change: 12.12 million rays/s. About the same (-0.5%).
